# dcjones/polee

Measured on AMD Instinct MI355X. Metric: approx-lik VI iters/sec, higher is better.
Workload: dtype f32

## Files before the change

include/polee_hip_debug.h:

```cpp
#ifndef POLEE_HIP_DEBUG_H
#define POLEE_HIP_DEBUG_H

#include "polee_hip.h"

#ifdef __cplusplus
extern "C" {
#endif

polee_status polee_debug_ptt_plan(const int32_t *node_parent_idxs, const int32_t *node_js, int32_t N,
                                  uint32_t *tour_code, int32_t *tour_tgt, int32_t *leaf_tid,
                                  int32_t *lo, int32_t *mid, int32_t *hi1, int32_t *max_depth);

typedef struct polee_psell_debug polee_psell_debug;
typedef struct {
    int64_t m, n, nnz, num_slices, num_tiles, padded_nnz, num_empty_rows;
    int64_t data_bytes, dict_len;
    int32_t max_row_nnz, max_tile_cols;
    const uint8_t *data;
    const uint32_t *slice_off;
    const uint32_t *tile_slice;
    const uint32_t *tile_dict;
    const uint32_t *dict;
    const uint32_t *row_order;
    const float *slice_ks;
    const uint8_t *slice_flags;
    int64_t num_tiles_a;
    int64_t num_tiles_a1;
    int64_t num_tiles_a1m;
    int64_t num_tiles_a2;
    const uint8_t *slice_w;
    int64_t num_tiles_s;
    int64_t stream_rows[8], stream_nnz[8], stream_bytes[8];
    int64_t csr_num_rows;
    const uint32_t *csr_rowptr;
    const uint32_t *csr_col;
    const float *csr_val;
    const uint32_t *csr_rows;
    int64_t single_num_rows;
    const uint32_t *single_rows;
    const float *single_cnt;
    double single_logsum;
} polee_psell_view;
polee_status polee_debug_psell_build(int64_t m, int64_t n, const void *colptr, int colptr_bytes,
                                     const uint32_t *rowval, const float *nzval,
                                     const int64_t *ks_or_null, polee_psell_debug **out);
polee_status polee_debug_psell_build_device(polee_ctx *ctx, int64_t m, int64_t n, const void *colptr, int colptr_bytes,
                                            const uint32_t *rowval, const float *nzval, const int64_t *ks_or_null,
                                            int device_stages, polee_psell_debug **out);
polee_status polee_debug_psell_view(const polee_psell_debug *p, polee_psell_view *view);
void polee_debug_psell_free(polee_psell_debug *p);

void polee_debug_device_cache_poison(int64_t *checked_blocks, int64_t *bad_blocks, int64_t *bad_words);

polee_status polee_debug_loglik_force_mixed(polee_loglik *ll, int on);

int64_t polee_debug_regression_num_stats(const polee_regression *reg);
polee_status polee_debug_regression_data_pass(polee_regression *reg, const float *noise, float *stats);
polee_status polee_debug_regression_prior_pass(polee_regression *reg, const float *stats, float *loss,
                                               float *grad_or_null);

polee_status polee_debug_comm_allreduce_ms(polee_comm *comm, int64_t count, int32_t reps, double *ms_avg);

polee_status polee_debug_fast_log(polee_ctx *ctx, const double *x, int64_t count, double *out);
polee_status polee_debug_fast_exp(polee_ctx *ctx, const double *x, int64_t count, double *out);

polee_status polee_debug_gibbs_assignments(polee_gibbs *g, int32_t chain, int32_t *z);

polee_status polee_debug_binomial(polee_ctx *ctx, const int64_t *N, const double *p, int64_t count, uint64_t seed, int64_t *out);

polee_status polee_debug_kmer_edges_count(polee_ctx *ctx_or_null, int64_t n, const uint64_t *sketches, int64_t *count);
polee_status polee_debug_kmer_edges_fill(polee_ctx *ctx_or_null, int64_t n, const uint64_t *sketches, int64_t capacity,
                                         uint32_t *u, uint32_t *v, uint32_t *mat, uint32_t *empt);

#ifdef __cplusplus
}
#endif
#endif
```

polee_amd/csrc/vi.hip:

```cpp
#include "loglik_internal.hpp"
#include "ptt_internal.hpp"
#include "vi_fused.hpp"
#include "comm_internal.hpp"
#include "rng.hpp"
#include "sampler_internal.hpp"

#include <cmath>

namespace polee {

struct NoiseSrc {
    const float *z0;
    uint64_t seed;
    int32_t K;
    int64_t nm1;
    __device__ inline float get(int step , int d, int64_t k) const
    {
        if (z0) return z0[((int64_t)(step - 1) * K + d) * nm1 + k];
        return philox_randn(seed, (uint32_t)step, (uint32_t)d, (uint32_t)k);
    }
    template <int KK>
    __device__ inline void get_all(int step, int64_t k, float (&z)[KK]) const
    {
        if (z0) {
#pragma unroll
            for (int d = 0; d < KK; ++d) z[d] = z0[((int64_t)(step - 1) * K + d) * nm1 + k];
            return;
        }
#pragma unroll
        for (int g = 0; g < (KK + 3) / 4; ++g) {
            float q[4];
            philox_randn4(seed, (uint32_t)step, (uint32_t)g, (uint32_t)k, q);
#pragma unroll
            for (int e = 0; e < 4; ++e)
                if (4 * g + e < KK) z[4 * g + e] = q[e];
        }
    }
};

__device__ inline float logistic_f32(float x) { return 1.0f / (1.0f + expf(-x)); }

__global__ void vi_trace_kernel(const double *lp, const double *ladj_el, const double *row_sums, int K, int idx,
                                double *elbo_trace, double *lp_trace)
{
    if (threadIdx.x != 0 || blockIdx.x != 0) return;
    const int d = K - 1;
    elbo_trace[idx] = (lp[d] + ladj_el[d * 2 + 0] + ladj_el[d * 2 + 1] + row_sums[d * 2 + 1]) / K;
    double s = 0.0;
    for (int i = 0; i < K; ++i) s += lp[i];
    lp_trace[idx] = s / K;
}

__global__ void vi_init_mu_kernel(const double *ys, int64_t nm1, float *mu, float *omega, float *alpha)
{
    const int64_t k = (int64_t)blockIdx.x * blockDim.x + threadIdx.x;
    if (k >= nm1) return;
    const double y = ys[k];
    mu[k] = (float)log(y / (1 - y));
    omega[k] = logf(0.1f);
    alpha[k] = 0.0f;
}

__global__ void aos_to_rows_f32_kernel(const float *in, int K, int64_t n, float *out, const uint32_t *index_of)
{
    const int64_t i = (int64_t)blockIdx.x * blockDim.x + threadIdx.x;
    if (i >= n * K) return;
    const int k = (int)(i / n);
    const int64_t j = i - (int64_t)k * n;
    out[i] = in[(index_of ? (int64_t)index_of[j] : j) * K + k];
}

__global__ void remap_u32_kernel(const uint32_t *src, const uint32_t *map, int64_t count, uint32_t *dst)
{
    const int64_t i = (int64_t)blockIdx.x * blockDim.x + threadIdx.x;
    if (i < count) dst[i] = map[src[i]];
}
template <typename T>
__global__ void gather_kernel(const T *src, const int32_t *idx, int64_t count, T *dst)
{
    const int64_t i = (int64_t)blockIdx.x * blockDim.x + threadIdx.x;
    if (i < count) dst[i] = src[idx[i]];
}

__global__ void vi_xgrad_rows_kernel(const float *g, const float *efflens, const double *csum, GenePrior gp, int K,
                                     int64_t n, double *out, const uint32_t *index_of)
{
    const int64_t i = (int64_t)blockIdx.x * blockDim.x + threadIdx.x;
    if (i >= n * K) return;
    const int k = (int)(i / n);
    const int64_t tid = index_of ? (int64_t)index_of[i - (int64_t)k * n] : i - (int64_t)k * n;
    double xg = (double)g[tid * K + k];
    if (efflens) xg -= (double)((float)n * (1.0f / efflens[tid])) / csum[k];
    if (gp.gene_of) {
        const int gene = gp.gene_of[tid];
        const int kg = gene >= 0 ? gp.gene_k[gene] : 0;
        const double c = csum[k], inv_l = (double)(1.0f / efflens[tid]);
        const double xlg = kg > 1 ? -(double)(kg - 1) / gp.gene_c[(size_t)gene * K + k] : 0.0;
        xg += xlg * (inv_l / c) + inv_l * (gp.M / (c * c));
    }
    out[i] = xg;
}

struct UniformLeafLoad {
    double val;
    __device__ dd operator()(int, int64_t) const { return dd_make(val); }
};
__global__ void vi_inverse_nodes_kernel(PttView v, const dd *C, double *ys)
{
    const int k = blockIdx.x * blockDim.x + threadIdx.x;
    if (k >= v.n - 1) return;
    const int lo = v.lo[k], mid = v.mid[k], hi1 = v.hi1[k];
    const double ur = dd_diff(C[mid], C[lo]);
    const double ul = dd_diff(C[hi1], C[mid]);
    ys[k] = ul / (ul + ur);
}

__global__ void sampler_y_kernel(const float *mu, const float *sigma, const float *alpha, NoiseSrc noise, int d_off, double y_eps,
                                 double *ys)
{
    const int64_t k = (int64_t)blockIdx.x * blockDim.x + threadIdx.x;
    const int d = blockIdx.y;
    if (k >= noise.nm1) return;
    const float z0 = noise.get(1, noise.z0 ? d : d + d_off, k);
    const float zs = sinhf(alpha[k] + asinhf(z0));
    double y = (double)logistic_f32(mu[k] + zs * sigma[k]);
    if (y_eps > 0.0) y = y < y_eps ? y_eps : (y > 1 - y_eps ? 1 - y_eps : y);
    ys[(int64_t)d * noise.nm1 + k] = y;
}

__global__ void export_noise_kernel(NoiseSrc noise, int step, float *out)
{
    const int64_t k = (int64_t)blockIdx.x * blockDim.x + threadIdx.x;
    const int d = blockIdx.y;
    if (k < noise.nm1) out[(int64_t)d * noise.nm1 + k] = noise.get(step, d, k);
}

}

using namespace polee;

struct polee_vi {
    polee_ctx *ctx = nullptr;
    polee_loglik *ll = nullptr;
    polee_ptt *t = nullptr;
    polee_vi_opts o;
    int32_t n = 0, K = 0;
    int32_t step = 0;
    int32_t ahead_step = 0;
    int32_t trace_cap = 0;
    polee_comm *comm = nullptr;
    DevBuf<float> d_efflens, d_mu, d_omega, d_alpha, d_mm, d_vm, d_mo, d_vo, d_ma, d_va, d_z0, d_x, d_g;
    DevBuf<float> d_zcur;
    DevBuf<float> d_y32;
    DevBuf<float> d_u32;
    DevBuf<uint32_t> d_open_ptr, d_open_code;
    bool leaf_order = false;
    DevBuf<uint32_t> d_index_of, d_dict_leaf, d_csr_col_leaf;
    DevBuf<float> d_single_leaf;
    LoglikRemap remap{nullptr, nullptr, nullptr, nullptr, false};
    DevBuf<double> d_ys, d_lyy, d_uleaf, d_part_c, d_part_ladj, d_csum, d_lp, d_ladj_el, d_rows, d_elbo, d_lptrace;
    DevBuf<dd> d_C;
    DevBuf<dd> d_chunk_bu;
    DevBuf<int32_t> d_node_start;
    DevBuf<uint32_t> d_need;
    DevBuf<float> d_H;
    int32_t bu_ch = 0;
    DevBuf<int> d_flag;
    DevBuf<int32_t> d_gene_of;
    DevBuf<int> d_gene_k;
    DevBuf<double> d_gene_c;
    int32_t num_genes = 0;
    double gene_M = 0.0;
    DevBuf<double> d_ygrad, d_xgrad_rows;
    DevBuf<float> d_mug, d_omg, d_alg, d_x_rows;

    NoiseSrc noise() const { return NoiseSrc{d_z0.p, o.seed, K, (int64_t)n - 1}; }
    polee_status one_step(bool apply, bool want_values, bool hook_outputs);
};

template <int K>
static polee_status vi_step_k(polee_vi *vi, bool apply, bool want_values, bool hook_outputs)
{
    polee_ctx *ctx = vi->ctx;
    polee_ptt *t = vi->t;
    const polee_vi_opts &o = vi->o;
    const int32_t n = vi->n;
    const int64_t nm1 = n - 1;
    const int step_num = vi->step + 1;
    hipStream_t st = ctx->stream;
    const PttView view = t->view();
    PttView lview = view;
    if (vi->leaf_order) lview.leaf_tid = nullptr;
    const LoglikRemap *remap = vi->leaf_order ? &vi->remap : nullptr;
    const uint32_t *index_of = vi->leaf_order ? vi->d_index_of.p : nullptr;
    const int nch_f = fwd_num_chunks(t->TL);
    const float *eff = o.use_efflen_jacobian ? vi->d_efflens.p : nullptr;
    VK<K> *chunk_f = reinterpret_cast<VK<K> *>(t->d_chunk.p);
    const NoiseSrc noise = vi->noise();

    if (want_values) POLEE_HIP_TRY(ctx, hipMemsetAsync(vi->d_ladj_el.p, 0, sizeof(double) * K * 2, st));
    if (nm1 > 0 && (vi->ahead_step != step_num || want_values)) {
        hipLaunchKernelGGL((vi_sample_k_kernel<K, NoiseSrc>), dim3((unsigned)ceil_div(nm1, 256)), dim3(256), 0, st,
                           vi->d_mu.p, vi->d_omega.p, vi->d_alpha.p, noise, step_num, vi->d_y32.p,
                           vi->d_zcur.p, want_values ? vi->d_ladj_el.p : nullptr);
        POLEE_KERNEL_CHECK(ctx);
    }
    const int own_f = nch_f <= 2048;
    const YRows ysrc{vi->d_y32.p, o.y_eps};
    const bool open_lists = vi->d_open_ptr.p != nullptr;
    static const bool xwin_fold = getenv("POLEE_VI_XWIN_FOLD") != nullptr && getenv("POLEE_NO_RING") == nullptr;
    const bool xwin_here = xwin_fold && !vi->leaf_order && !vi->ll->force_mixed && vi->ll->d_xwin.p && vi->ll->d_tslot_ptr.p && vi->ll->host.num_tiles_s > 0;
    if (open_lists) {
    } else if (nch_f > 1) {
        hipLaunchKernelGGL((vi_fwd_reduce_kernel<K, YRows>), dim3(nch_f), dim3(SCAN_THREADS), 0, st, view, ysrc, chunk_f);
        if (!own_f) hipLaunchKernelGGL((scan_spine_kernel<VK<K>>), dim3(1), dim3(SCAN_THREADS), 0, st, chunk_f, nch_f);
    } else {
        POLEE_HIP_TRY(ctx, hipMemsetAsync(chunk_f, 0, sizeof(VK<K>), st));
    }
    if (want_values) {
        hipLaunchKernelGGL((vi_fwd_apply_kernel<K, YRows, float, true>), dim3(nch_f), dim3(SCAN_THREADS), 0, st, lview, ysrc, chunk_f,
                           vi->d_u32.p, vi->d_x.p, vi->d_g.p, eff, (float)o.y_eps, (float)(1.0 - o.y_eps),
                           eff ? vi->d_part_c.p : nullptr, want_values ? vi->d_part_ladj.p : nullptr, nch_f > 1 ? own_f : 0,
                           (const uint32_t *)vi->d_open_ptr.p, (const uint32_t *)vi->d_open_code.p,
                           xwin_here ? (const uint32_t *)vi->ll->d_tslot_ptr.p : nullptr, xwin_here ? (const uint32_t *)vi->ll->d_tslot.p : nullptr,
                           xwin_here ? vi->ll->d_xwin.p : nullptr,
                           remap && remap->singles_in_g ? (const float *)vi->d_single_leaf.p : nullptr);
    } else {
        hipLaunchKernelGGL((vi_fwd_apply_kernel<K, YRows, float, false>), dim3(nch_f), dim3(SCAN_THREADS), 0, st, lview, ysrc, chunk_f,
                           vi->d_u32.p, vi->d_x.p, vi->d_g.p, eff, (float)o.y_eps, (float)(1.0 - o.y_eps),
                           eff ? vi->d_part_c.p : nullptr, want_values ? vi->d_part_ladj.p : nullptr, nch_f > 1 ? own_f : 0,
                           (const uint32_t *)vi->d_open_ptr.p, (const uint32_t *)vi->d_open_code.p,
                           xwin_here ? (const uint32_t *)vi->ll->d_tslot_ptr.p : nullptr, xwin_here ? (const uint32_t *)vi->ll->d_tslot.p : nullptr,
                           xwin_here ? vi->ll->d_xwin.p : nullptr,
                           remap && remap->singles_in_g ? (const float *)vi->d_single_leaf.p : nullptr);
    }
    POLEE_KERNEL_CHECK(ctx);
    if (want_values) POLEE_HIP_TRY(ctx, hipMemsetAsync(vi->d_lp.p, 0, sizeof(double) * PSELL_MAX_K, st));
    {
        const bool det_saved = vi->ll->deterministic;
        if (o.deterministic > 0 || (o.deterministic == 0 && vi->comm && vi->comm->nranks > 1)) vi->ll->deterministic = true;
        vi->ll->side_part = eff ? vi->d_part_c.p : nullptr;
        vi->ll->side_nparts = nch_f;
        vi->ll->side_out = vi->d_csum.p;
        vi->ll->side_done = false;
        const polee_status ls = loglik_eval_device(vi->ll, vi->d_x.p, K, vi->d_g.p, want_values ? vi->d_lp.p : nullptr, xwin_here, remap);
        vi->ll->deterministic = det_saved;
        const bool side_done = vi->ll->side_done;
        vi->ll->side_part = nullptr;
        POLEE_TRY(ls);
        if (eff && !side_done)
            hipLaunchKernelGGL((vi_csum_finish_kernel<K>), dim3(1), dim3(256), 0, st, (const double *)vi->d_part_c.p, nch_f, vi->d_csum.p);
    }
    if (vi->comm) {
        POLEE_TRY(comm_allreduce_device(vi->comm, vi->d_g.p, (size_t)n * K, false));
        if (want_values) POLEE_TRY(comm_allreduce_device(vi->comm, vi->d_lp.p, (size_t)K, true));
    }
    GenePrior gp{nullptr, nullptr, nullptr, 0.0};
    if (vi->num_genes > 0) {
        gp = GenePrior{vi->d_gene_of.p, vi->d_gene_k.p, vi->d_gene_c.p, vi->gene_M};
        POLEE_HIP_TRY(ctx, hipMemsetAsync(vi->d_gene_c.p, 0, sizeof(double) * (size_t)vi->num_genes * K, st));
        hipLaunchKernelGGL((vi_gene_sums_kernel<K>), dim3((unsigned)ceil_div((int64_t)n, 256)), dim3(256), 0, st, vi->d_x.p,
                           vi->d_efflens.p, vi->d_part_c.p, nch_f, (int64_t)n, gp, vi->d_gene_c.p);
    }
    AdamConsts a;
    a.lr = std::max(o.adam_min_learning_rate,
                    o.adam_initial_learning_rate * std::exp(-o.adam_learning_rate_decay * (double)(step_num - 1)));
    a.rm = o.adam_rm;
    a.rv = o.adam_rv;
    a.eps = o.adam_eps;
    a.m_denom = 1 - std::pow(o.adam_rm, (double)step_num);
    a.v_denom = 1 - std::pow(o.adam_rv, (double)step_num);
    a.inv_m_denom = 1.0 / a.m_denom;
    a.inv_v_denom = 1.0 / a.v_denom;
    a.max_mu = o.max_mu_step;
    a.max_omega = o.max_omega_step;
    a.max_alpha = o.max_alpha_step;
    a.first = step_num == 1;
    const bool sample_next = apply && !(o.z0 && step_num + 1 > o.num_steps);
    const UpdArgs ua{vi->d_y32.p, vi->d_mu.p, vi->d_omega.p, vi->d_alpha.p, vi->d_mm.p, vi->d_vm.p, vi->d_mo.p, vi->d_vo.p,
                     vi->d_ma.p, vi->d_va.p, a, apply ? 1 : 0, vi->d_flag.p, hook_outputs ? vi->d_ygrad.p : nullptr,
                     hook_outputs ? vi->d_mug.p : nullptr, hook_outputs ? vi->d_omg.p : nullptr,
                     hook_outputs ? vi->d_alg.p : nullptr, sample_next ? 1 : 0, o.y_eps, vi->d_zcur.p, step_num};
    {
        const int nch_bu = (int)ceil_div((int64_t)n, bu_ch<K>());
        VD<K> *chunk_bu = reinterpret_cast<VD<K> *>(vi->d_chunk_bu.p);
        const BwdArgs<K> ba{lview, vi->d_u32.p, vi->d_g.p, eff, vi->d_csum.p, gp, chunk_bu, vi->d_C.p, (const uint32_t *)vi->d_need.p,
                            (const int32_t *)vi->d_node_start.p, vi->d_H.p};
        hipLaunchKernelGGL((vi_bwd_local_kernel<K>), dim3(nch_bu), dim3(256), 0, st, ba);
        if (nm1 > 0) {
            hipLaunchKernelGGL((vi_bwd_spine_kernel<K>), dim3(1), dim3(64 * K), 0, st, chunk_bu, nch_bu);
            hipLaunchKernelGGL((vi_update_k_kernel<K, NoiseSrc>), dim3((unsigned)ceil_div(nm1, 256)), dim3(256), 0, st, view,
                               (const float *)vi->d_H.p, (const VD<K> *)chunk_bu, (const dd *)vi->d_C.p, ua, noise);
        }
        if (nm1 > 0) vi->ahead_step = apply ? (sample_next ? step_num + 1 : 0) : step_num;
    }
    POLEE_KERNEL_CHECK(ctx);
    if (want_values) {
        hipLaunchKernelGGL((vi_values_finish_kernel<K>), dim3(1), dim3(256), 0, st, vi->d_part_ladj.p, nch_f,
                           eff ? vi->d_csum.p : nullptr, vi->d_rows.p);
        POLEE_KERNEL_CHECK(ctx);
    }
    if (hook_outputs) {
        hipLaunchKernelGGL(vi_xgrad_rows_kernel, dim3((unsigned)ceil_div((int64_t)n * K, 256)), dim3(256), 0, st,
                           vi->d_g.p, eff, vi->d_csum.p, gp, K, (int64_t)n, vi->d_xgrad_rows.p, index_of);
        POLEE_KERNEL_CHECK(ctx);
    }
    if (want_values && apply && vi->step < vi->trace_cap) {
        hipLaunchKernelGGL(vi_trace_kernel, dim3(1), dim3(64), 0, st, vi->d_lp.p, vi->d_ladj_el.p, vi->d_rows.p, K,
                           vi->step, vi->d_elbo.p, vi->d_lptrace.p);
        POLEE_KERNEL_CHECK(ctx);
    }
    if (apply) ++vi->step;
    return POLEE_OK;
}

polee_status polee_vi::one_step(bool apply, bool want_values, bool hook_outputs)
{
    POLEE_TRY(t->reserve(K));
    if (o.z0 && step + 1 > o.num_steps)
        return fail(ctx, POLEE_ERR_BAD_ARG, "caller-supplied z0 covers only %d steps", o.num_steps);
    switch (K) {
        case 1: return vi_step_k<1>(this, apply, want_values, hook_outputs);
        case 2: return vi_step_k<2>(this, apply, want_values, hook_outputs);
        case 3: return vi_step_k<3>(this, apply, want_values, hook_outputs);
        case 4: return vi_step_k<4>(this, apply, want_values, hook_outputs);
        case 5: return vi_step_k<5>(this, apply, want_values, hook_outputs);
        case 6: return vi_step_k<6>(this, apply, want_values, hook_outputs);
        case 7: return vi_step_k<7>(this, apply, want_values, hook_outputs);
        case 8: return vi_step_k<8>(this, apply, want_values, hook_outputs);
    }
    return fail(ctx, POLEE_ERR_BAD_ARG, "num_mc_samples must be in 1..8");
}

namespace polee {

static polee_status sampler_draw_device(polee_ptt *t, const float *mu, const float *sigma, const float *alpha,
                                        const float *z0, int32_t ndraws, uint64_t seed, DevBuf<float> &d_all,
                                        double y_eps = 0.0)
{
    polee_ctx *ctx = t->ctx;
    if (!mu || !sigma || !alpha || ndraws < 1) return fail(ctx, POLEE_ERR_BAD_ARG, "bad argument");
    if (t->T != 1) return fail(ctx, POLEE_ERR_BAD_ARG, "the sampler needs a single tree");
    const size_t n = t->n, nm1 = n - 1;
    DevBuf<float> d_mu, d_sigma, d_alpha, d_z0;
    POLEE_TRY(d_mu.upload(ctx, mu, nm1));
    POLEE_TRY(d_sigma.upload(ctx, sigma, nm1));
    POLEE_TRY(d_alpha.upload(ctx, alpha, nm1));
    POLEE_TRY(d_all.alloc(ctx, (size_t)ndraws * n));
    for (int32_t b0 = 0; b0 < ndraws; b0 += SAMPLER_BLOCK) {
        const int32_t B = std::min(SAMPLER_BLOCK, ndraws - b0);
        if (z0) POLEE_TRY(d_z0.upload(ctx, z0 + (size_t)b0 * nm1, (size_t)B * nm1));
        POLEE_TRY(sampler_block_device(t, d_mu.p, d_sigma.p, d_alpha.p, z0 ? d_z0.p : nullptr, seed, (uint64_t)b0, 0, B, y_eps,
                                       d_all.p + (size_t)b0 * n, (int64_t)n));
    }
    return POLEE_OK;
}

polee_status sampler_block_device(polee_ptt *t, const float *d_mu, const float *d_sigma, const float *d_alpha, const float *d_z0,
                                  uint64_t seed, uint64_t b0, int32_t r0, int32_t B, double y_eps, float *d_xs, int64_t xs_rs)
{
    polee_ctx *ctx = t->ctx;
    const size_t nm1 = (size_t)t->n - 1;
    POLEE_TRY(t->reserve(B));
    NoiseSrc noise{d_z0, sampler_block_seed(seed, b0), B, (int64_t)nm1};
    if (nm1 > 0) {
        hipLaunchKernelGGL(sampler_y_kernel, dim3((unsigned)ceil_div(nm1, 256), B), dim3(256), 0, ctx->stream, d_mu, d_sigma,
                           d_alpha, noise, (int)r0, y_eps, t->d_ys.p);
        POLEE_KERNEL_CHECK(ctx);
    }
    FwdOut o;
    o.xs = d_xs;
    o.xs_rs = xs_rs;
    return ptt_forward_device(t, t->d_ys.p, B, o);
}

__global__ void sampler_mean_kernel(const float *xs, int ndraws, int64_t n, float *pm)
{
    const int64_t j = (int64_t)blockIdx.x * blockDim.x + threadIdx.x;
    if (j >= n) return;
    float acc = 0.0f;
    for (int k = 0; k < ndraws; ++k) acc += fminf(fmaxf(xs[(int64_t)k * n + j], 1e-15f), 0.9999999f);
    pm[j] = acc / (float)ndraws;
}

__global__ void x0_sums_kernel(const float *xs, const float *efflens, int64_t n, double *sums)
{
    __shared__ double smd[4];
    const int d = blockIdx.y;
    double q = 0.0;
    for (int64_t j = (int64_t)blockIdx.x * blockDim.x + threadIdx.x; j < n; j += (int64_t)gridDim.x * blockDim.x)
        q += (double)(xs[(int64_t)d * n + j] / efflens[j]);
    q = block_sum_f64(q, smd);
    if (threadIdx.x == 0) atomicAdd(&sums[d], q);
}
__global__ void x0_mean_kernel(const float *xs, const float *efflens, const double *sums, int ndraws, int64_t n, float *x0)
{
    const int64_t j = (int64_t)blockIdx.x * blockDim.x + threadIdx.x;
    if (j >= n) return;
    float acc = 0.0f;
    for (int d = 0; d < ndraws; ++d) acc += (xs[(int64_t)d * n + j] / efflens[j]) / (float)sums[d];
    x0[j] = acc / (float)ndraws;
}

constexpr int SAMPLER_MAX_Q = 8;
struct QuantileSpec {
    int nq;
    int j[SAMPLER_MAX_Q];
    double gamma[SAMPLER_MAX_Q];
};
__global__ __launch_bounds__(64) void sampler_quantile_kernel(const float *xs, int ndraws, int64_t n, QuantileSpec spec,
                                                              int in_lds, float *out)
{
    extern __shared__ float col[];
    const int64_t jj = (int64_t)blockIdx.x * 64 + threadIdx.x;
    const int64_t j = jj < n ? jj : n - 1;
    if (in_lds)
        for (int k = 0; k < ndraws; ++k) col[k * 64 + threadIdx.x] = xs[(int64_t)k * n + j];
    auto at = [&](int k) { return in_lds ? col[k * 64 + threadIdx.x] : xs[(int64_t)k * n + j]; };
    float a[SAMPLER_MAX_Q], b[SAMPLER_MAX_Q];
#pragma unroll
    for (int i = 0; i < SAMPLER_MAX_Q; ++i) a[i] = b[i] = 0.0f;
    for (int e = 0; e < ndraws; ++e) {
        const float ve = at(e);
        int rank = 0;
        for (int i = 0; i < ndraws; ++i) {
            const float vi = at(i);
            rank += (vi < ve || (vi == ve && i < e)) ? 1 : 0;
        }
#pragma unroll
        for (int i = 0; i < SAMPLER_MAX_Q; ++i)
            if (i < spec.nq) {
                if (rank == spec.j[i] - 1) a[i] = ve;
                if (rank == spec.j[i] || ndraws == 1) b[i] = ve;
            }
    }
    if (jj < n)
#pragma unroll
        for (int i = 0; i < SAMPLER_MAX_Q; ++i)
            if (i < spec.nq) out[(int64_t)i * n + j] = (float)((double)a[i] + spec.gamma[i] * (double)(b[i] - a[i]));
}

}
using namespace polee;

extern "C" {

void polee_vi_default_opts(polee_vi_opts *o)
{
    if (!o) return;
    memset(o, 0, sizeof(*o));
    o->num_steps = 500;
    o->num_mc_samples = 6;
    o->use_efflen_jacobian = 1;
    o->gradonly = 1;
    o->seed = 123456789ull;
    o->z0 = nullptr;
    o->y_eps = 1e-10;
    o->adam_initial_learning_rate = 1.0;
    o->adam_learning_rate_decay = 2e-2;
    o->adam_min_learning_rate = 1e-3;
    o->adam_eps = 1e-8;
    o->adam_rv = 0.9;
    o->adam_rm = 0.7;
    o->max_mu_step = 2e-1;
    o->max_omega_step = 2e-1;
    o->max_alpha_step = 2e-2;
    o->profile = 0;
    o->deterministic = 0;
    o->gene_of = nullptr;
}

static thread_local bool g_vi_plain_order = false;

polee_status polee_vi_create(polee_loglik *ll, polee_ptt *t, const float *efflens, const polee_vi_opts *opts,
                             polee_vi **out)
{
    if (!ll || !t) return fail(nullptr, POLEE_ERR_BAD_ARG, "null handle");
    polee_ctx *ctx = ll->ctx;
    POLEE_TRY(use_device(ctx));
    if (t->ctx != ctx) return fail(ctx, POLEE_ERR_BAD_ARG, "likelihood and tree belong to different contexts");
    if (!out || !efflens) return fail(ctx, POLEE_ERR_BAD_ARG, "null argument");
    if (t->T != 1) return fail(ctx, POLEE_ERR_BAD_ARG, "the VI loop needs a single tree");
    if ((int64_t)t->n != ll->n)
        return fail(ctx, POLEE_ERR_BAD_ARG, "tree has %d leaves but X has %lld transcripts", t->n, (long long)ll->n);
    polee_vi_opts o;
    if (opts)
        o = *opts;
    else
        polee_vi_default_opts(&o);
    if (o.num_mc_samples < 1 || o.num_mc_samples > PSELL_MAX_K)
        return fail(ctx, POLEE_ERR_BAD_ARG, "num_mc_samples must be in 1..8");
    if (o.num_steps < 0) return fail(ctx, POLEE_ERR_BAD_ARG, "num_steps must be >= 0");
    if (!(o.y_eps > 0.0 && o.y_eps < 0.5)) return fail(ctx, POLEE_ERR_BAD_ARG, "y_eps must lie in (0, 0.5) (LIKAP_Y_EPS = 1e-10)");
    std::vector<int> gene_k;
    double gene_M = 0.0;
    if (o.gene_of) {
        if (!o.use_efflen_jacobian)
            return fail(ctx, POLEE_ERR_BAD_ARG, "gene_of needs use_efflen_jacobian (gene_noninformative_prior! works on the "
                                                "xls of the effective-length adjustment, likelihood.jl:114-159)");
        int32_t ng = 0;
        for (int64_t i = 0; i < ll->n; ++i) {
            if (o.gene_of[i] < -1) return fail(ctx, POLEE_ERR_BAD_ARG, "gene_of[%lld] = %d", (long long)i, o.gene_of[i]);
            ng = std::max(ng, o.gene_of[i] + 1);
        }
        gene_k.assign((size_t)ng, 0);
        for (int64_t i = 0; i < ll->n; ++i)
            if (o.gene_of[i] >= 0) ++gene_k[o.gene_of[i]];
        for (int k : gene_k)
            if (k > 1) gene_M += (double)(k - 1);
    }
    polee_vi *vi = new (std::nothrow) polee_vi();
    if (!vi) return fail(ctx, POLEE_ERR_OOM, "out of host memory");
    vi->ctx = ctx;
    vi->ll = ll;
    vi->t = t;
    ctx_retain(ctx);
    loglik_retain(ll);
    ptt_retain(t);
    vi->o = o;
    vi->n = t->n;
    vi->K = o.num_mc_samples;
    ll->profile = o.profile != 0;
    ll->prof_every = o.profile > 1 ? o.profile : 1;
    const size_t n = vi->n, nm1 = std::max<size_t>(n - 1, 1), K = vi->K;
    polee_status s = POLEE_OK;
    auto A = [&](polee_status r) {
        if (s == POLEE_OK) s = r;
    };
    A(vi->d_efflens.upload(ctx, efflens, n));
    for (DevBuf<float> *b : {&vi->d_mu, &vi->d_omega, &vi->d_alpha, &vi->d_mm, &vi->d_vm, &vi->d_mo, &vi->d_vo,
                             &vi->d_ma, &vi->d_va, &vi->d_mug, &vi->d_omg, &vi->d_alg})
        A(b->alloc(ctx, nm1));
    A(vi->d_x.alloc(ctx, n * K));
    A(vi->d_zcur.alloc(ctx, nm1 * K));
    A(vi->d_y32.alloc(ctx, nm1 * K));
    A(vi->d_g.alloc(ctx, n * K));
    A(vi->d_x_rows.alloc(ctx, n * K));
    A(vi->d_ys.alloc(ctx, nm1));
    if (g_vi_plain_order) A(vi->d_lyy.alloc(ctx, nm1 * 2));
    A(vi->d_u32.alloc(ctx, n * K));
    if (g_vi_plain_order) A(vi->d_uleaf.alloc(ctx, n));
    A(vi->d_C.alloc(ctx, (n + 1) * K));
    {
        const size_t nch = (size_t)std::max(scan_num_chunks(3 * (int64_t)n - 2), 1);
        A(vi->d_part_c.alloc(ctx, nch * K));
        A(vi->d_part_ladj.alloc(ctx, nch * K));
        A(vi->d_csum.alloc(ctx, 2 * PSELL_MAX_K));
    }
    {
        const PttPlan &pl = t->plans[0];
        const int CH = K <= 6 ? bu_ch<6>() : bu_ch<8>();
        vi->bu_ch = CH;
        const int nch_bu = (int)ceil_div((int64_t)n, CH);
        std::vector<int32_t> node_start((size_t)nch_bu + 1, (int32_t)(n - 1));
        std::vector<uint32_t> need((n + 1 + 31) / 32 + 1, 0u);
        bool monotone = true;
        int c = 0;
        for (size_t k = 0; k + 1 < n; ++k) {
            if (k > 0 && pl.lo[k] < pl.lo[k - 1]) monotone = false;
            for (; c <= pl.lo[k] / CH; ++c) node_start[(size_t)c] = (int32_t)k;
            const int64_t end = std::min<int64_t>(((int64_t)pl.lo[k] / CH + 1) * CH, (int64_t)n);
            if (pl.hi1[k] > end)
                for (int32_t b : {pl.lo[k], pl.mid[k], pl.hi1[k]}) need[(size_t)b >> 5] |= 1u << (b & 31);
        }
        if (!monotone) A(fail(ctx, POLEE_ERR_BAD_ARG, "tree plan: internal nodes are not in DFS pre-order"));
        A(vi->d_node_start.upload(ctx, node_start));
        A(vi->d_need.upload(ctx, need));
        A(vi->d_chunk_bu.alloc(ctx, ((size_t)nch_bu + 1) * K));
        A(vi->d_H.alloc(ctx, 2 * K * nm1));
        if (s == POLEE_OK && hipMemsetAsync(vi->d_C.p, 0, sizeof(dd) * (n + 1) * K, ctx->stream) != hipSuccess)
            A(fail(ctx, POLEE_ERR_HIP, "memset failed"));
    }
    {
        static const bool no_open = getenv("POLEE_VI_NO_OPEN_LISTS") != nullptr;
        const std::vector<uint32_t> &code = t->plans[0].tour_code;
        const int64_t TL = t->TL;
        const size_t limit = (size_t)8 << 20;
        std::vector<uint32_t> optr, ocode;
        const bool ok = !no_open && t->T == 1 && (int64_t)code.size() == TL && build_open_lists(code.data(), TL, FWD_CHUNK, limit, optr, ocode);
        if (ok) {
            if (ocode.empty()) ocode.push_back(4u | TOUR_LEAF);
            A(vi->d_open_ptr.upload(ctx, optr));
            A(vi->d_open_code.upload(ctx, ocode));
        }
    }
    A(vi->d_ygrad.alloc(ctx, nm1 * K));
    A(vi->d_xgrad_rows.alloc(ctx, n * K));
    A(vi->d_lp.alloc(ctx, PSELL_MAX_K));
    A(vi->d_ladj_el.alloc(ctx, PSELL_MAX_K * 2));
    A(vi->d_rows.alloc(ctx, PSELL_MAX_K * 2));
    A(vi->d_flag.alloc(ctx, 1));
    if (!gene_k.empty()) {
        vi->num_genes = (int32_t)gene_k.size();
        vi->gene_M = gene_M;
        A(vi->d_gene_of.upload(ctx, o.gene_of, n));
        A(vi->d_gene_k.upload(ctx, gene_k));
        A(vi->d_gene_c.alloc(ctx, gene_k.size() * K));
    }
    static const bool no_leaf_env = getenv("POLEE_VI_NO_LEAF_ORDER") != nullptr;
    if (!no_leaf_env && !g_vi_plain_order && n > 1 && t->plans.size() == 1 && t->plans[0].tid_pos.size() == n) {
        const PttPlan &pl = t->plans[0];
        std::vector<uint32_t> index_of(n);
        std::vector<float> eff_leaf(n);
        for (size_t j = 0; j < n; ++j) index_of[j] = (uint32_t)pl.tid_pos[j];
        for (size_t pos = 0; pos < n; ++pos) eff_leaf[pos] = efflens[pl.leaf_tid[pos]];
        A(vi->d_index_of.upload(ctx, index_of));
        A(vi->d_efflens.upload(ctx, eff_leaf));
        if (!gene_k.empty()) {
            std::vector<int32_t> gene_leaf(n);
            for (size_t pos = 0; pos < n; ++pos) gene_leaf[pos] = o.gene_of[pl.leaf_tid[pos]];
            A(vi->d_gene_of.upload(ctx, gene_leaf));
        }
        A(vi->d_dict_leaf.alloc(ctx, (size_t)std::max<int64_t>(ll->dict_len, 1)));
        if (ll->csr_nnz > 0) A(vi->d_csr_col_leaf.alloc(ctx, (size_t)ll->csr_nnz));
        if (ll->has_singles) A(vi->d_single_leaf.alloc(ctx, n));
        if (s == POLEE_OK) {
            hipStream_t st0 = ctx->stream;
            if (ll->dict_len > 0)
                hipLaunchKernelGGL(remap_u32_kernel, dim3((unsigned)ceil_div(ll->dict_len, 256)), dim3(256), 0, st0,
                                   (const uint32_t *)ll->d_dict.p, (const uint32_t *)vi->d_index_of.p, ll->dict_len, vi->d_dict_leaf.p);
            if (ll->csr_nnz > 0)
                hipLaunchKernelGGL(remap_u32_kernel, dim3((unsigned)ceil_div(ll->csr_nnz, 256)), dim3(256), 0, st0,
                                   (const uint32_t *)ll->d_csr_col.p, (const uint32_t *)vi->d_index_of.p, ll->csr_nnz, vi->d_csr_col_leaf.p);
            if (ll->has_singles)
                hipLaunchKernelGGL(gather_kernel<float>, dim3((unsigned)ceil_div((int64_t)n, 256)), dim3(256), 0, st0,
                                   (const float *)ll->d_single_cnt.p, (const int32_t *)t->d_leaf_tid.p, (int64_t)n, vi->d_single_leaf.p);
            if (hipGetLastError() != hipSuccess) A(fail(ctx, POLEE_ERR_HIP, "leaf-order tables: kernel launch failed"));
            vi->leaf_order = true;
            vi->remap = LoglikRemap{vi->d_dict_leaf.p, ll->has_singles ? vi->d_single_leaf.p : nullptr,
                                    ll->csr_nnz > 0 ? vi->d_csr_col_leaf.p : nullptr, vi->d_index_of.p, ll->has_singles};
        }
    }
    vi->o.gene_of = nullptr;
    vi->trace_cap = o.gradonly ? 0 : std::max(o.num_steps, 1);
    if (!o.gradonly) {
        A(vi->d_elbo.alloc(ctx, vi->trace_cap));
        A(vi->d_lptrace.alloc(ctx, vi->trace_cap));
    }
    if (o.z0 && o.num_steps > 0) A(vi->d_z0.upload(ctx, o.z0, (size_t)o.num_steps * K * (n - 1)));
    vi->o.z0 = o.z0;
    A(t->reserve((int32_t)K));
    if (s != POLEE_OK) {
        polee_vi_destroy(vi);
        return s;
    }
    hipStream_t st = ctx->stream;
    hipError_t e = hipMemsetAsync(vi->d_flag.p, 0, sizeof(int), st);
    if (e == hipSuccess) e = hipMemsetAsync(vi->d_rows.p, 0, sizeof(double) * PSELL_MAX_K * 2, st);
    for (DevBuf<float> *b : {&vi->d_mm, &vi->d_vm, &vi->d_mo, &vi->d_vo, &vi->d_ma, &vi->d_va})
        if (e == hipSuccess) e = hipMemsetAsync(b->p, 0, sizeof(float) * nm1, st);
    if (e != hipSuccess) {
        polee_vi_destroy(vi);
        return fail(ctx, POLEE_ERR_HIP, "memset failed: %s", hipGetErrorString(e));
    }
    if (n > 1) {
        UniformLeafLoad load{(double)(1.0f / (float)n)};
        LeafPrefixEmit emit{(int32_t)n, t->d_C.p};
        e = run_scan_partial<dd>(st, 1, n, t->d_chunk.p, nullptr, load, emit);
        if (e == hipSuccess) {
            hipLaunchKernelGGL(vi_inverse_nodes_kernel, dim3((unsigned)ceil_div(n - 1, 256)), dim3(256), 0, st,
                               t->view(), t->d_C.p, vi->d_ys.p);
            hipLaunchKernelGGL(vi_init_mu_kernel, dim3((unsigned)ceil_div(n - 1, 256)), dim3(256), 0, st, vi->d_ys.p,
                               (int64_t)n - 1, vi->d_mu.p, vi->d_omega.p, vi->d_alpha.p);
            e = hipGetLastError();
        }
        if (e == hipSuccess) e = hipStreamSynchronize(st);
        if (e != hipSuccess) {
            polee_vi_destroy(vi);
            return fail(ctx, POLEE_ERR_HIP, "initialisation failed: %s", hipGetErrorString(e));
        }
    }
    *out = vi;
    return POLEE_OK;
}

void polee_vi_destroy(polee_vi *vi)
{
    if (!vi) return;
    polee_ctx *ctx = vi->ctx;
    polee_loglik *ll = vi->ll;
    polee_ptt *t = vi->t;
    polee_comm *comm = vi->comm;
    if (ctx) {
        (void)hipSetDevice(ctx->device);
        (void)hipStreamSynchronize(ctx->stream);
    }
    delete vi;
    polee_comm_destroy(comm);
    loglik_release(ll);
    ptt_release(t);
    ctx_release(ctx);
}

polee_status polee_vi_set_comm(polee_vi *vi, polee_comm *comm)
{
    if (!vi) return fail(nullptr, POLEE_ERR_BAD_ARG, "null handle");
    if (comm && comm->ctx != vi->ctx)
        return fail(vi->ctx, POLEE_ERR_BAD_ARG, "communicator and fit belong to different contexts");
    if (comm) ++comm->refs;
    polee_comm_destroy(vi->comm);
    vi->comm = comm;
    return POLEE_OK;
}

polee_status polee_vi_run(polee_vi *vi, int32_t nsteps)
{
    if (!vi) return fail(nullptr, POLEE_ERR_BAD_ARG, "null handle");
    POLEE_TRY(use_device(vi->ctx));
    vi->ll->profile = vi->o.profile != 0;
    vi->ll->prof_every = vi->o.profile > 1 ? vi->o.profile : 1;
    for (int32_t i = 0; i < nsteps; ++i) POLEE_TRY(vi->one_step(true, !vi->o.gradonly, false));
    return POLEE_OK;
}

polee_status polee_vi_sync(polee_vi *vi)
{
    if (!vi) return fail(nullptr, POLEE_ERR_BAD_ARG, "null handle");
    polee_ctx *ctx = vi->ctx;
    POLEE_TRY(use_device(ctx));
    int flag = 0;
    POLEE_TRY(vi->d_flag.download(ctx, &flag, 1));
    if (vi->ll->profile) POLEE_TRY(vi->ll->profile_collect());
    if (flag != 0)
        return fail(ctx, POLEE_ERR_NONFINITE, "non-finite gradient at VI step %d (likelihood-approximation.jl:559)",
                    flag);
    return POLEE_OK;
}

polee_status polee_vi_get_params(polee_vi *vi, float *mu, float *omega, float *alpha)
{
    if (!vi) return fail(nullptr, POLEE_ERR_BAD_ARG, "null handle");
    polee_ctx *ctx = vi->ctx;
    POLEE_TRY(use_device(ctx));
    const size_t nm1 = vi->n - 1;
    if (mu) POLEE_TRY(vi->d_mu.download(ctx, mu, nm1));
    if (omega) POLEE_TRY(vi->d_omega.download(ctx, omega, nm1));
    if (alpha) POLEE_TRY(vi->d_alpha.download(ctx, alpha, nm1));
    return POLEE_OK;
}

polee_status polee_vi_set_params(polee_vi *vi, const float *mu, const float *omega, const float *alpha)
{
    if (!vi) return fail(nullptr, POLEE_ERR_BAD_ARG, "null handle");
    polee_ctx *ctx = vi->ctx;
    POLEE_TRY(use_device(ctx));
    const size_t nm1 = vi->n - 1;
    if (mu) POLEE_TRY(vi->d_mu.upload(ctx, mu, nm1));
    if (omega) POLEE_TRY(vi->d_omega.upload(ctx, omega, nm1));
    if (alpha) POLEE_TRY(vi->d_alpha.upload(ctx, alpha, nm1));
    vi->ahead_step = 0;
    return POLEE_OK;
}

polee_status polee_vi_get_stats(polee_vi *vi, polee_vi_stats *stats)
{
    if (!vi || !stats) return fail(nullptr, POLEE_ERR_BAD_ARG, "null argument");
    polee_ctx *ctx = vi->ctx;
    POLEE_TRY(use_device(ctx));
    memset(stats, 0, sizeof(*stats));
    stats->steps_done = vi->step;
    int flag = 0;
    POLEE_TRY(vi->d_flag.download(ctx, &flag, 1));
    stats->nonfinite_step = flag;
    if (vi->ll->profile) POLEE_TRY(vi->ll->profile_collect());
    stats->loglik_kernel_launches = vi->ll->prof_launches;
    stats->loglik_kernel_ms_avg = vi->ll->prof_launches ? vi->ll->prof_ms_total / vi->ll->prof_launches : 0.0;
    stats->loglik_pass_ms_avg = vi->ll->prof_launches ? vi->ll->prof_pass_ms_total / vi->ll->prof_launches : 0.0;
    if (!vi->o.gradonly && vi->step > 0 && vi->step <= vi->trace_cap) {
        POLEE_HIP_TRY(ctx, hipMemcpyAsync(&stats->last_elbo, vi->d_elbo.p + (vi->step - 1), sizeof(double),
                                          hipMemcpyDeviceToHost, ctx->stream));
        POLEE_HIP_TRY(ctx, hipMemcpyAsync(&stats->last_lp_mean, vi->d_lptrace.p + (vi->step - 1), sizeof(double),
                                          hipMemcpyDeviceToHost, ctx->stream));
        POLEE_HIP_TRY(ctx, hipStreamSynchronize(ctx->stream));
    }
    return POLEE_OK;
}

polee_status polee_vi_get_trace(polee_vi *vi, double *elbo, double *lp_mean)
{
    if (!vi) return fail(nullptr, POLEE_ERR_BAD_ARG, "null handle");
    polee_ctx *ctx = vi->ctx;
    POLEE_TRY(use_device(ctx));
    if (vi->o.gradonly) return fail(ctx, POLEE_ERR_BAD_ARG, "no trace is recorded in gradonly mode");
    const size_t cnt = std::min(vi->step, vi->trace_cap);
    if (elbo) POLEE_TRY(vi->d_elbo.download(ctx, elbo, cnt));
    if (lp_mean) POLEE_TRY(vi->d_lptrace.download(ctx, lp_mean, cnt));
    return POLEE_OK;
}

#ifdef POLEE_VI_STAMPS
polee_status polee_debug_vi_stamps(unsigned long long *out)
{
    return hipMemcpyFromSymbol(out, HIP_SYMBOL(polee::g_vi_stamps), sizeof(unsigned long long) * 4 * 2048 * 8) == hipSuccess ? POLEE_OK : POLEE_ERR_HIP;
}
#endif

polee_status polee_vi_export_noise(polee_vi *vi, int32_t step, float *z0)
{
    if (!vi || !z0 || step < 1) return fail(nullptr, POLEE_ERR_BAD_ARG, "bad argument");
    polee_ctx *ctx = vi->ctx;
    POLEE_TRY(use_device(ctx));
    const int64_t nm1 = vi->n - 1;
    if (nm1 < 1) return POLEE_OK;
    if (vi->o.z0 && step > vi->o.num_steps) return fail(ctx, POLEE_ERR_BAD_ARG, "step beyond the supplied noise");
    DevBuf<float> tmp;
    POLEE_TRY(tmp.alloc(ctx, (size_t)vi->K * nm1));
    hipLaunchKernelGGL(export_noise_kernel, dim3((unsigned)ceil_div(nm1, 256), vi->K), dim3(256), 0, ctx->stream,
                       vi->noise(), step, tmp.p);
    POLEE_KERNEL_CHECK(ctx);
    return tmp.download(ctx, z0, (size_t)vi->K * nm1);
}

polee_status polee_vi_eval_gradients(polee_vi *vi, float *xs, double *x_grad, double *y_grad, float *mu_grad,
                                     float *omega_grad, float *alpha_grad, double *lp, double *ladj)
{
    if (!vi) return fail(nullptr, POLEE_ERR_BAD_ARG, "null handle");
    polee_ctx *ctx = vi->ctx;
    POLEE_TRY(use_device(ctx));
    const size_t n = vi->n, nm1 = n - 1, K = vi->K;
    POLEE_TRY(vi->one_step(false, true, true));
    if (xs) {
        hipLaunchKernelGGL(aos_to_rows_f32_kernel, dim3((unsigned)ceil_div(n * K, 256)), dim3(256), 0, ctx->stream,
                           vi->d_x.p, (int)K, (int64_t)n, vi->d_x_rows.p, vi->leaf_order ? (const uint32_t *)vi->d_index_of.p : nullptr);
        POLEE_KERNEL_CHECK(ctx);
        POLEE_TRY(vi->d_x_rows.download(ctx, xs, n * K));
    }
    if (x_grad) POLEE_TRY(vi->d_xgrad_rows.download(ctx, x_grad, n * K));
    if (y_grad) POLEE_TRY(vi->d_ygrad.download(ctx, y_grad, nm1 * K));
    if (mu_grad) POLEE_TRY(vi->d_mug.download(ctx, mu_grad, nm1));
    if (omega_grad) POLEE_TRY(vi->d_omg.download(ctx, omega_grad, nm1));
    if (alpha_grad) POLEE_TRY(vi->d_alg.download(ctx, alpha_grad, nm1));
    if (lp) POLEE_TRY(vi->d_lp.download(ctx, lp, K));
    if (ladj) {
        std::vector<double> el(K * 2), rs(K * 2);
        POLEE_TRY(vi->d_ladj_el.download(ctx, el.data(), K * 2));
        POLEE_TRY(vi->d_rows.download(ctx, rs.data(), K * 2));
        for (size_t d = 0; d < K; ++d) ladj[d] = el[d * 2] + el[d * 2 + 1] + rs[d * 2 + 1];
    }
    return POLEE_OK;
}

polee_status polee_vi_fit(polee_loglik *ll, polee_ptt *t, const float *efflens, const polee_vi_opts *opts, float *mu,
                          float *omega, float *alpha, polee_vi_stats *stats)
{
    polee_vi *vi = nullptr;
    POLEE_TRY(polee_vi_create(ll, t, efflens, opts, &vi));
    polee_status s = polee_vi_run(vi, vi->o.num_steps);
    if (s == POLEE_OK) s = polee_vi_sync(vi);
    if (s == POLEE_OK) s = polee_vi_get_params(vi, mu, omega, alpha);
    if (s == POLEE_OK && stats) s = polee_vi_get_stats(vi, stats);
    polee_vi_destroy(vi);
    return s;
}

polee_status polee_optimize_ptt(polee_loglik *ll, polee_ptt *t, const float *efflens, int32_t num_steps, float *xs,
                                float *zs_out)
{
    if (!ll || !t || !efflens || !xs || num_steps < 0) return fail(nullptr, POLEE_ERR_BAD_ARG, "bad argument");
    polee_vi_opts o;
    polee_vi_default_opts(&o);
    o.num_steps = num_steps;
    o.num_mc_samples = 1;
    polee_vi *vi = nullptr;
    g_vi_plain_order = true;
    const polee_status cs = polee_vi_create(ll, t, efflens, &o, &vi);
    g_vi_plain_order = false;
    POLEE_TRY(cs);
    polee_ctx *ctx = vi->ctx;
    hipStream_t st = ctx->stream;
    const int32_t n = vi->n;
    const int64_t nm1 = n - 1;
    const PttView view = t->view();
    const int nch_f = fwd_num_chunks(t->TL), nch_b = scan_num_chunks(n);
    VK<1> *chunk_f = reinterpret_cast<VK<1> *>(t->d_chunk.p);
    VD<1> *chunk_b = reinterpret_cast<VD<1> *>(t->d_chunk.p);
    polee_status rc = POLEE_OK;
    auto forward = [&]() -> polee_status {
        hipLaunchKernelGGL(point_sample_kernel, dim3((unsigned)ceil_div(nm1, 256)), dim3(256), 0, st, vi->d_mu.p, nm1,
                           vi->d_ys.p, vi->d_lyy.p);
        if (nch_f > 1) {
            hipLaunchKernelGGL((vi_fwd_reduce_kernel<1, LogRows>), dim3(nch_f), dim3(SCAN_THREADS), 0, st, view, LogRows{vi->d_lyy.p}, chunk_f);
            hipLaunchKernelGGL((scan_spine_kernel<VK<1>>), dim3(1), dim3(SCAN_THREADS), 0, st, chunk_f, nch_f);
        } else {
            POLEE_HIP_TRY(ctx, hipMemsetAsync(chunk_f, 0, sizeof(VK<1>), st));
        }
        hipLaunchKernelGGL((vi_fwd_apply_kernel<1, LogRows, double, false>), dim3(nch_f), dim3(SCAN_THREADS), 0, st, view, LogRows{vi->d_lyy.p}, chunk_f,
                           vi->d_uleaf.p, vi->d_x.p, vi->d_g.p, vi->d_efflens.p, (float)o.y_eps, (float)(1.0 - o.y_eps),
                           vi->d_part_c.p, (double *)nullptr, 0, (const uint32_t *)nullptr, (const uint32_t *)nullptr,
                           (const uint32_t *)nullptr, (const uint32_t *)nullptr, (float *)nullptr, (const float *)nullptr);
        POLEE_KERNEL_CHECK(ctx);
        return POLEE_OK;
    };
    for (int step_num = 1; step_num <= num_steps && rc == POLEE_OK && nm1 > 0; ++step_num) {
        rc = forward();
        if (rc != POLEE_OK) break;
        rc = loglik_eval_device(ll, vi->d_x.p, 1, vi->d_g.p, nullptr);
        if (rc != POLEE_OK) break;
        const GenePrior no_gp{nullptr, nullptr, nullptr, 0.0};
        hipLaunchKernelGGL((vi_bwd_reduce_kernel<1>), dim3(nch_b), dim3(SCAN_THREADS), 0, st, view, vi->d_uleaf.p,
                           vi->d_g.p, vi->d_efflens.p, vi->d_part_c.p, nch_f, vi->d_csum.p, no_gp, chunk_b);
        hipLaunchKernelGGL((scan_spine_kernel<VD<1>>), dim3(1), dim3(SCAN_THREADS), 0, st, chunk_b, nch_b);
        hipLaunchKernelGGL((vi_bwd_apply_kernel<1>), dim3(nch_b), dim3(SCAN_THREADS), 0, st, view, vi->d_uleaf.p,
                           vi->d_g.p, vi->d_efflens.p, vi->d_csum.p, no_gp, chunk_b, vi->d_C.p, 0);
        AdamConsts a;
        a.lr = std::max(o.adam_min_learning_rate,
                        o.adam_initial_learning_rate * std::exp(-o.adam_learning_rate_decay * (double)(step_num - 1)));
        a.rm = o.adam_rm;
        a.rv = o.adam_rv;
        a.eps = o.adam_eps;
        a.m_denom = 1 - std::pow(o.adam_rm, (double)step_num);
        a.v_denom = 1 - std::pow(o.adam_rv, (double)step_num);
        a.inv_m_denom = 1.0 / a.m_denom;
        a.inv_v_denom = 1.0 / a.v_denom;
        a.max_mu = 1e-1;
        a.max_omega = a.max_alpha = 0.0;
        a.first = step_num == 1;
        hipLaunchKernelGGL(point_update_kernel, dim3((unsigned)ceil_div(nm1, 256)), dim3(256), 0, st, view, vi->d_ys.p,
                           vi->d_C.p, vi->d_mu.p, vi->d_mm.p, vi->d_vm.p, a, vi->d_flag.p, step_num);
        hipError_t e = hipGetLastError();
        if (e != hipSuccess) rc = fail(ctx, POLEE_ERR_HIP, "kernel launch failed: %s", hipGetErrorString(e));
    }
    if (rc == POLEE_OK) rc = forward();
    if (rc == POLEE_OK) rc = polee_vi_sync(vi);
    if (rc == POLEE_OK) rc = vi->d_x.download(ctx, xs, n);
    if (rc == POLEE_OK && zs_out) rc = vi->d_mu.download(ctx, zs_out, nm1);
    polee_vi_destroy(vi);
    return rc;
}

polee_status polee_sampler_draw(polee_ptt *t, const float *mu, const float *sigma, const float *alpha,
                                const float *z0, int32_t ndraws, uint64_t seed, float *xs)
{
    if (!t) return fail(nullptr, POLEE_ERR_BAD_ARG, "null tree");
    polee_ctx *ctx = t->ctx;
    POLEE_TRY(use_device(ctx));
    if (!xs) return fail(ctx, POLEE_ERR_BAD_ARG, "bad argument");
    DevBuf<float> d_all;
    POLEE_TRY(sampler_draw_device(t, mu, sigma, alpha, z0, ndraws, seed, d_all));
    return d_all.download(ctx, xs, (size_t)ndraws * t->n);
}

polee_status polee_sampler_initial_values(polee_ptt *t, const float *mu, const float *sigma, const float *alpha,
                                          const float *efflens, const float *z0, int32_t ndraws, uint64_t seed, float *x0)
{
    if (!t) return fail(nullptr, POLEE_ERR_BAD_ARG, "null tree");
    polee_ctx *ctx = t->ctx;
    POLEE_TRY(use_device(ctx));
    if (!x0 || !efflens) return fail(ctx, POLEE_ERR_BAD_ARG, "bad argument");
    DevBuf<float> d_all, d_l, d_x0;
    DevBuf<double> d_sums;
    POLEE_TRY(sampler_draw_device(t, mu, sigma, alpha, z0, ndraws, seed, d_all, 1e-10 ));
    const int64_t n = t->n;
    POLEE_TRY(d_l.upload(ctx, efflens, (size_t)n));
    POLEE_TRY(d_x0.alloc(ctx, (size_t)n));
    POLEE_TRY(d_sums.alloc(ctx, (size_t)ndraws));
    POLEE_HIP_TRY(ctx, hipMemsetAsync(d_sums.p, 0, sizeof(double) * ndraws, ctx->stream));
    hipLaunchKernelGGL(x0_sums_kernel, dim3((unsigned)std::min<int64_t>(ceil_div(n, 256), 256), (unsigned)ndraws), dim3(256), 0,
                       ctx->stream, d_all.p, d_l.p, n, d_sums.p);
    hipLaunchKernelGGL(x0_mean_kernel, dim3((unsigned)ceil_div(n, 256)), dim3(256), 0, ctx->stream, d_all.p, d_l.p, d_sums.p,
                       ndraws, n, d_x0.p);
    POLEE_KERNEL_CHECK(ctx);
    return d_x0.download(ctx, x0, (size_t)n);
}

polee_status polee_sampler_posterior_mean(polee_ptt *t, const float *mu, const float *sigma, const float *alpha,
                                          const float *z0, int32_t ndraws, uint64_t seed, float *pm)
{
    if (!t) return fail(nullptr, POLEE_ERR_BAD_ARG, "null tree");
    polee_ctx *ctx = t->ctx;
    POLEE_TRY(use_device(ctx));
    if (!pm) return fail(ctx, POLEE_ERR_BAD_ARG, "bad argument");
    DevBuf<float> d_all, d_pm;
    POLEE_TRY(sampler_draw_device(t, mu, sigma, alpha, z0, ndraws, seed, d_all));
    POLEE_TRY(d_pm.alloc(ctx, (size_t)t->n));
    hipLaunchKernelGGL(sampler_mean_kernel, dim3((unsigned)ceil_div(t->n, 256)), dim3(256), 0, ctx->stream, d_all.p,
                       ndraws, (int64_t)t->n, d_pm.p);
    POLEE_KERNEL_CHECK(ctx);
    return d_pm.download(ctx, pm, (size_t)t->n);
}

polee_status polee_sampler_quantiles(polee_ptt *t, const float *mu, const float *sigma, const float *alpha,
                                     const float *z0, int32_t ndraws, uint64_t seed, const double *qs, int32_t nq,
                                     float *quantiles)
{
    if (!t) return fail(nullptr, POLEE_ERR_BAD_ARG, "null tree");
    polee_ctx *ctx = t->ctx;
    POLEE_TRY(use_device(ctx));
    if (!qs || !quantiles || nq < 1 || nq > SAMPLER_MAX_Q) return fail(ctx, POLEE_ERR_BAD_ARG, "1..%d quantiles", SAMPLER_MAX_Q);
    QuantileSpec spec{};
    spec.nq = nq;
    for (int i = 0; i < nq; ++i) {
        if (!(qs[i] >= 0.0 && qs[i] <= 1.0)) return fail(ctx, POLEE_ERR_BAD_ARG, "quantile %g outside [0, 1]", qs[i]);
        const double aleph = (double)(ndraws - 1) * qs[i] + 1.0;
        const int j = ndraws == 1 ? 1 : std::min(std::max((int)aleph, 1), ndraws - 1);
        spec.j[i] = j;
        spec.gamma[i] = std::min(std::max(aleph - j, 0.0), 1.0);
    }
    DevBuf<float> d_all, d_q;
    POLEE_TRY(sampler_draw_device(t, mu, sigma, alpha, z0, ndraws, seed, d_all));
    const int64_t n = t->n;
    POLEE_TRY(d_q.alloc(ctx, (size_t)nq * n));
    const bool in_lds = (size_t)ndraws * 64 * sizeof(float) <= 48 * 1024;
    hipLaunchKernelGGL(sampler_quantile_kernel, dim3((unsigned)ceil_div(n, 64)), dim3(64),
                       in_lds ? (size_t)ndraws * 64 * sizeof(float) : 0, ctx->stream, d_all.p, ndraws, n, spec,
                       in_lds ? 1 : 0, d_q.p);
    POLEE_KERNEL_CHECK(ctx);
    return d_q.download(ctx, quantiles, (size_t)nq * n);
}

}
```

polee_amd/csrc/vi_fused.hpp:

```cpp
#pragma once
#include "ptt_internal.hpp"

namespace polee {

#ifdef POLEE_VI_STAMPS
__device__ unsigned long long g_vi_stamps[4][2048][8];
#define VI_STAMP(kern, slot)                                                                                        \
    do {                                                                                                            \
        asm volatile("s_waitcnt vmcnt(0) lgkmcnt(0)" ::: "memory");                                                 \
        if (threadIdx.x == 0 && blockIdx.x < 2048) g_vi_stamps[kern][blockIdx.x][slot] = __builtin_amdgcn_s_memrealtime(); \
    } while (0)
#else
#define VI_STAMP(kern, slot) do {} while (0)
#endif

template <int K>
struct VK {
    double v[K];
};
template <int K>
struct VD {
    dd v[K];
};
template <int K>
struct ScanOps<VK<K>> {
    __device__ static VK<K> zero()
    {
        VK<K> r;
#pragma unroll
        for (int d = 0; d < K; ++d) r.v[d] = 0.0;
        return r;
    }
    __device__ static VK<K> add(const VK<K> &a, const VK<K> &b)
    {
        VK<K> r;
#pragma unroll
        for (int d = 0; d < K; ++d) r.v[d] = a.v[d] + b.v[d];
        return r;
    }
    __device__ static VK<K> shfl_up(const VK<K> &a, int dist)
    {
        VK<K> r;
#pragma unroll
        for (int d = 0; d < K; ++d) r.v[d] = __shfl_up(a.v[d], dist, 64);
        return r;
    }
    template <int CTRL, int ROW_MASK>
    __device__ static VK<K> dpp(const VK<K> &a)
    {
        VK<K> r;
#pragma unroll
        for (int d = 0; d < K; ++d) r.v[d] = dpp_f64<CTRL, ROW_MASK>(a.v[d]);
        return r;
    }
};
template <int K>
struct ScanOps<VD<K>> {
    __device__ static VD<K> zero()
    {
        VD<K> r;
#pragma unroll
        for (int d = 0; d < K; ++d) r.v[d] = dd{0.0, 0.0};
        return r;
    }
    __device__ static VD<K> add(const VD<K> &a, const VD<K> &b)
    {
        VD<K> r;
#pragma unroll
        for (int d = 0; d < K; ++d) r.v[d] = dd_add(a.v[d], b.v[d]);
        return r;
    }
    __device__ static VD<K> shfl_up(const VD<K> &a, int dist)
    {
        VD<K> r;
#pragma unroll
        for (int d = 0; d < K; ++d) r.v[d] = dd{__shfl_up(a.v[d].hi, dist, 64), __shfl_up(a.v[d].lo, dist, 64)};
        return r;
    }
    template <int CTRL, int ROW_MASK>
    __device__ static VD<K> dpp(const VD<K> &a)
    {
        VD<K> r;
#pragma unroll
        for (int d = 0; d < K; ++d) r.v[d] = dd{dpp_f64<CTRL, ROW_MASK>(a.v[d].hi), dpp_f64<CTRL, ROW_MASK>(a.v[d].lo)};
        return r;
    }
};

template <int K>
__device__ inline void block_sum_vec(double (&v)[K], double *smem)
{
    const int lane = threadIdx.x & 63, wave = threadIdx.x >> 6;
#pragma unroll
    for (int d = 0; d < K; ++d) {
        const double s = wave_inclusive_scan<double>(v[d]);
        if (lane == 63) smem[wave * K + d] = s;
    }
    __syncthreads();
    if (threadIdx.x < K) {
        const double s = smem[threadIdx.x] + smem[K + threadIdx.x] + smem[2 * K + threadIdx.x] + smem[3 * K + threadIdx.x];
        smem[threadIdx.x] = s;
    }
    __syncthreads();
#pragma unroll
    for (int d = 0; d < K; ++d) v[d] = smem[d];
    __syncthreads();
}

template <int K>
__device__ inline void store_vec_by_thread(const double (&v)[K], double *out)
{
#pragma unroll
    for (int d = 0; d < K; ++d)
        if (threadIdx.x == d) out[d] = v[d];
}

__device__ inline float sinh_asinh(float sa, float ca, float z0) { return fmaf(sa, sqrtf(fmaf(z0, z0, 1.0f)), ca * z0); }

__device__ inline double clamped_y(float y32, double y_eps)
{
    const double y = (double)y32;
    return y < y_eps ? y_eps : (y > 1 - y_eps ? 1 - y_eps : y);
}
__device__ inline double clamped_y_pos(float y32, double y_eps, double one_m_eps)
{
    const double y = (double)y32;
    return fmin(fmax(y, y_eps), one_m_eps);
}
template <int K, typename Noise>
__device__ inline void sample_node(float m, float om, float al, const Noise &noise, int step, int64_t k,
                                   float *__restrict__ y32, float *__restrict__ zcur, double *lsum)
{
    const float sigma = expf(om);
    const float sa = sinhf(al), ca = coshf(al);
    float zall[K];
    noise.template get_all<K>(step, k, zall);
#pragma unroll
    for (int d = 0; d < K; ++d) {
        const float z0 = zall[d];
        zcur[k * K + d] = z0;
        const float zs = sinh_asinh(sa, ca, z0);
        const float yf = 1.0f / (1.0f + expf(-(m + zs * sigma)));
        if (lsum) {
            const double y = (double)yf;
            lsum[d] = 0.5 * (double)log1pf(zs * zs) - 0.5 * (double)log1pf(z0 * z0);
            lsum[K + d] = log((double)sigma * y * (1 - y));
        }
        y32[k * K + d] = yf;
    }
}

template <int K, typename Noise>
__global__ __launch_bounds__(256) void vi_sample_k_kernel(const float *__restrict__ mu, const float *__restrict__ omega,
                                                         const float *__restrict__ alpha, Noise noise, int step,
                                                         float *__restrict__ y32, float *__restrict__ zcur,
                                                         double *__restrict__ ladj_out)
{
    __shared__ double smem[4 * 2 * K];
    const int64_t k = (int64_t)blockIdx.x * blockDim.x + threadIdx.x;
    double lsum[2 * K];
#pragma unroll
    for (int d = 0; d < 2 * K; ++d) lsum[d] = 0.0;
    if (k < noise.nm1)
        sample_node<K, Noise>(mu[k], omega[k], alpha[k], noise, step, k, y32, zcur, ladj_out ? lsum : nullptr);
    if (ladj_out) {
        block_sum_vec<2 * K>(lsum, smem);
#pragma unroll
        for (int i = 0; i < 2 * K; ++i)
            if (threadIdx.x == i) atomicAdd(&ladj_out[(i % K) * 2 + i / K], lsum[i]);
    }
}

struct LogRows {
    const double *lyy;
    template <int K>
    __device__ inline double edge_one(uint32_t k, uint32_t left, int d) const { return lyy[((size_t)k * 2 + left) * K + d]; }
    template <int K>
    __device__ inline void edge(uint32_t k, uint32_t left, double (&e)[K]) const
    {
        const double *p = lyy + ((size_t)k * 2 + left) * K;
#pragma unroll
        for (int d = 0; d < K; ++d) e[d] = p[d];
    }
};
struct YRows {
    const float *y32;
    double y_eps;
    template <int K>
    __device__ inline double edge_one(uint32_t k, uint32_t left, int d) const
    {
        const double y = clamped_y_pos(y32[(size_t)k * K + d], y_eps, 1.0 - y_eps);
        return fast_log_pos(left ? y : 1.0 - y);
    }
    template <int K>
    __device__ inline void edge(uint32_t k, uint32_t left, double (&e)[K]) const
    {
        const float *p = y32 + (size_t)k * K;
        const double hi = 1.0 - y_eps;
#pragma unroll
        for (int d = 0; d < K; ++d) {
            const double y = clamped_y_pos(p[d], y_eps, hi);
            e[d] = fast_log_pos(left ? y : 1.0 - y);
        }
    }
};

constexpr int FWD_ITEMS = 2;
constexpr int FWD_CHUNK = SCAN_THREADS * FWD_ITEMS;
inline int fwd_num_chunks(int64_t len) { return (int)((len + FWD_CHUNK - 1) / FWD_CHUNK); }

template <int K, typename Src>
__device__ inline VK<K> tour_value(uint32_t code, const Src &src, VK<K> &edge)
{
    VK<K> val;
    const uint32_t type = code & 3u;
    if (code & 4u) {
#pragma unroll
        for (int d = 0; d < K; ++d) edge.v[d] = 0.0;
    } else {
        src.template edge<K>(code >> 4, (code >> 3) & 1u, edge.v);
    }
#pragma unroll
    for (int d = 0; d < K; ++d) val.v[d] = type == TOUR_ENTER ? edge.v[d] : (type == TOUR_EXIT ? -edge.v[d] : 0.0);
    return val;
}

template <typename T>
__device__ inline T chunk_prefix(const T *__restrict__ chunk_sums, int chunk, T *smem)
{
    T acc = ScanOps<T>::zero();
    for (int i = threadIdx.x; i < chunk; i += SCAN_THREADS) acc = ScanOps<T>::add(acc, chunk_sums[i]);
    T tot;
    (void)block_exclusive_scan<T>(acc, smem, &tot);
    return tot;
}

template <int K, typename Src>
__global__ __launch_bounds__(SCAN_THREADS) void vi_fwd_reduce_kernel(PttView v, Src lyy,
                                                                    VK<K> *__restrict__ chunk_sums)
{
    __shared__ VK<K> smem[SCAN_THREADS / 64];
    const int64_t base = (int64_t)blockIdx.x * FWD_CHUNK + (int64_t)threadIdx.x * FWD_ITEMS;
    VK<K> acc = ScanOps<VK<K>>::zero(), edge;
#pragma unroll
    for (int j = 0; j < FWD_ITEMS; ++j)
        if (base + j < v.TL) acc = ScanOps<VK<K>>::add(acc, tour_value<K, Src>(v.tour_code[base + j], lyy, edge));
    VK<K> tot;
    (void)block_exclusive_scan<VK<K>>(acc, smem, &tot);
    if (threadIdx.x == 0) chunk_sums[blockIdx.x] = tot;
}

template <int K, typename Src, typename UT, bool LADJ>
__global__ __launch_bounds__(SCAN_THREADS) void vi_fwd_apply_kernel(PttView v, Src lyy,
                                                                   const VK<K> *__restrict__ chunk_offsets,
                                                                   UT *__restrict__ uleaf, float *__restrict__ xs,
                                                                   float *__restrict__ g,
                                                                   const float *__restrict__ efflens, float clamp_lo,
                                                                   float clamp_hi, double *__restrict__ part_c,
                                                                   double *__restrict__ part_ladj, int own_prefix,
                                                                   const uint32_t *__restrict__ open_ptr,
                                                                   const uint32_t *__restrict__ open_code,
                                                                   const uint32_t *__restrict__ tslot_ptr,
                                                                   const uint32_t *__restrict__ tslot,
                                                                   float *__restrict__ xwin,
                                                                   const float *__restrict__ single_cnt)
{
    __shared__ VK<K> smem[SCAN_THREADS / 64];
    __shared__ double smd[4 * K];
    __shared__ double spre[K];
    __shared__ double smd2[LADJ ? 4 * K : 1];
    constexpr int XW_INLINE = 12, XW_DEFER = 48;
    __shared__ uint32_t xw_tid[XW_DEFER];
    __shared__ float xw_val[XW_DEFER][K];
    __shared__ int xw_count;
    if (xwin && threadIdx.x == 0) xw_count = 0;
    if (xwin) __syncthreads();
    const int64_t base = (int64_t)blockIdx.x * FWD_CHUNK + (int64_t)threadIdx.x * FWD_ITEMS;
    VK<K> w[FWD_ITEMS];
    uint32_t code[FWD_ITEMS];
    int tgt[FWD_ITEMS];
#pragma unroll
    for (int j = 0; j < FWD_ITEMS; ++j) {
        code[j] = base + j < v.TL ? v.tour_code[base + j] : (4u | TOUR_LEAF);
        tgt[j] = base + j < v.TL ? v.tour_tgt[base + j] : 0;
    }
    VI_STAMP(0, 0);
    const int lane = threadIdx.x & 63;
    uint32_t ob = 0, oe = 0;
    if (open_ptr) {
        ob = open_ptr[blockIdx.x];
        oe = open_ptr[blockIdx.x + 1];
    }
    const int wave = threadIdx.x >> 6;
    const uint32_t ocode0 = ob + lane < oe ? open_code[ob + lane] : (4u | TOUR_LEAF);
    VK<K> acc = ScanOps<VK<K>>::zero();
    float inv_l_[FWD_ITEMS], sc_[FWD_ITEMS];
    int ltid[FWD_ITEMS];
#pragma unroll
    for (int j = 0; j < FWD_ITEMS; ++j) {
        acc = ScanOps<VK<K>>::add(acc, tour_value<K, Src>(code[j], lyy, w[j]));
        const bool leaf = (code[j] & 3u) == TOUR_LEAF && base + j < v.TL;
        ltid[j] = leaf ? (v.leaf_tid ? v.leaf_tid[tgt[j]] : tgt[j]) : 0;
        inv_l_[j] = leaf && efflens ? 1.0f / efflens[ltid[j]] : 0.0f;
        sc_[j] = leaf && single_cnt ? single_cnt[ltid[j]] : 0.0f;
    }
    VI_STAMP(0, 1);
    if (open_ptr) {
#pragma unroll
        for (int dd_ = 0; dd_ < (K + 3) / 4; ++dd_) {
            const int d = wave + 4 * dd_;
            if (d < K) {
                double pre = (ocode0 & 4u) ? 0.0 : lyy.template edge_one<K>(ocode0 >> 4, (ocode0 >> 3) & 1u, d);
                for (uint32_t e = ob + 64 + lane; e < oe; e += 64) {
                    const uint32_t oc = open_code[e];
                    pre += lyy.template edge_one<K>(oc >> 4, (oc >> 3) & 1u, d);
                }
                pre = wave_inclusive_scan<double>(pre);
                if (lane == 63) spre[d] = pre;
            }
        }
    }
    VI_STAMP(0, 2);
    VK<K> tot;
    VK<K> off = block_exclusive_scan<VK<K>>(acc, smem, &tot);
    VI_STAMP(0, 3);
    if (open_ptr) {
#pragma unroll
        for (int d = 0; d < K; ++d) off.v[d] += spre[d];
    } else {
        off = ScanOps<VK<K>>::add(own_prefix ? chunk_prefix<VK<K>>(chunk_offsets, blockIdx.x, smem) : chunk_offsets[blockIdx.x], off);
    }
    double pc[K], pl[K];
#pragma unroll
    for (int d = 0; d < K; ++d) pc[d] = pl[d] = 0.0;
#pragma unroll
    for (int j = 0; j < FWD_ITEMS; ++j) {
        const uint32_t tj = code[j] & 3u;
#pragma unroll
        for (int d = 0; d < K; ++d) off.v[d] = tj == TOUR_ENTER ? off.v[d] + w[j].v[d] : (tj == TOUR_EXIT ? off.v[d] - w[j].v[d] : off.v[d]);
        const VK<K> &inc = off;
        if (base + j < v.TL) {
            const uint32_t type = code[j] & 3u;
            if (type == TOUR_LEAF) {
                const int pos = tgt[j];
                const int tid = ltid[j];
                const float inv_l = inv_l_[j];
                const float sc = sc_[j];
#pragma unroll
                for (int d = 0; d < K; ++d) {
                    const double u = fast_exp(inc.v[d] + w[j].v[d]);
                    uleaf[(size_t)pos * K + d] = (UT)u;
                    float x = (float)u;
                    x = (float)fmax((double)x, 1e-16);
                    x = fminf(fmaxf(x, clamp_lo), clamp_hi);
                    xs[(size_t)tid * K + d] = x;
                    g[(size_t)tid * K + d] = sc != 0.0f ? sc / x : 0.0f;
                    pc[d] += (double)(x * inv_l);
                }
                if (xwin) {
                    const uint32_t sb = tslot_ptr[tid], se = tslot_ptr[tid + 1];
                    int q = -1;
                    if (se - sb > (uint32_t)XW_INLINE) q = atomicAdd(&xw_count, 1);
                    if (q >= 0 && q < XW_DEFER) {
                        xw_tid[q] = (uint32_t)tid;
#pragma unroll
                        for (int d = 0; d < K; ++d) xw_val[q][d] = xs[(size_t)tid * K + d];
                    } else {
                        for (uint32_t e = sb; e < se; ++e) {
                            float *w = xwin + (size_t)tslot[e] * K;
#pragma unroll
                            for (int d = 0; d < K; ++d) w[d] = xs[(size_t)tid * K + d];
                        }
                    }
                }
            } else if (LADJ && type == TOUR_ENTER) {
#pragma unroll
                for (int d = 0; d < K; ++d) pl[d] += inc.v[d];
            }
        }
    }
    if (xwin) {
        __syncthreads();
        const int cnt = min(xw_count, XW_DEFER);
        for (int q = 0; q < cnt; ++q) {
            const uint32_t tid = xw_tid[q], sb = tslot_ptr[tid], se = tslot_ptr[tid + 1];
            for (uint32_t e = sb * K + threadIdx.x; e < se * K; e += SCAN_THREADS) {
                const uint32_t slot = e / K, d = e - slot * K;
                xwin[(size_t)tslot[slot] * K + d] = xw_val[q][d];
            }
        }
    }
    VI_STAMP(0, 4);
    if (part_c || LADJ) {
#pragma unroll
        for (int d = 0; d < K; ++d) {
            const double a = wave_inclusive_scan<double>(pc[d]);
            const double b = LADJ ? wave_inclusive_scan<double>(pl[d]) : 0.0;
            if (lane == 63) {
                smd[wave * K + d] = a;
                if (LADJ) smd2[wave * K + d] = b;
            }
        }
        __syncthreads();
        if ((int)threadIdx.x < K) {
            const int d = threadIdx.x;
            if (part_c) part_c[(size_t)blockIdx.x * K + d] = ((smd[d] + smd[K + d]) + smd[2 * K + d]) + smd[3 * K + d];
            if (LADJ) part_ladj[(size_t)blockIdx.x * K + d] = ((smd2[d] + smd2[K + d]) + smd2[2 * K + d]) + smd2[3 * K + d];
        }
    }
    VI_STAMP(0, 5);
}

struct GenePrior {
    const int32_t *gene_of;
    const int *gene_k;
    const double *gene_c;
    double M;
};

template <int K>
__device__ inline void bwd_values(const PttView &v, int64_t pos, const double *__restrict__ uleaf,
                                  const float *__restrict__ g, const float *__restrict__ efflens,
                                  const double *csum, const GenePrior &gp, VD<K> &a)
{
    const int tid = v.leaf_tid ? v.leaf_tid[pos] : (int)pos;
    const float inv_lf = efflens ? 1.0f / efflens[tid] : 0.0f;
    const float nl = (float)v.n * inv_lf;
    int gene = -1, kg = 0;
    if (gp.gene_of) {
        gene = gp.gene_of[tid];
        kg = gene >= 0 ? gp.gene_k[gene] : 0;
    }
#pragma unroll
    for (int d = 0; d < K; ++d) {
        double xg = (double)g[(size_t)tid * K + d];
        if (efflens) xg -= (double)nl / csum[d];
        if (gp.gene_of) {
            const double c = csum[d], inv_l = (double)inv_lf;
            const double xlg = kg > 1 ? -(double)(kg - 1) / gp.gene_c[(size_t)gene * K + d] : 0.0;
            xg += xlg * (inv_l / c) + inv_l * (gp.M / (c * c));
        }
        a.v[d] = dd_make(uleaf[(size_t)pos * K + d] * xg);
    }
}

template <int K>
__global__ __launch_bounds__(256) void vi_gene_sums_kernel(const float *__restrict__ xs, const float *__restrict__ efflens,
                                                          const double *__restrict__ part_c, int nchunks_fwd, int64_t n,
                                                          GenePrior gp, double *__restrict__ gene_c)
{
    __shared__ double smd[4 * K];
    double c[K];
#pragma unroll
    for (int d = 0; d < K; ++d) c[d] = 0.0;
    for (int ch = threadIdx.x; ch < nchunks_fwd; ch += 256)
#pragma unroll
        for (int d = 0; d < K; ++d) c[d] += part_c[(size_t)ch * K + d];
    block_sum_vec<K>(c, smd);
    const int64_t tid = (int64_t)blockIdx.x * 256 + threadIdx.x;
    if (tid >= n) return;
    const int gene = gp.gene_of[tid];
    if (gene < 0 || gp.gene_k[gene] <= 1) return;
    const float inv_l = 1.0f / efflens[tid];
#pragma unroll
    for (int d = 0; d < K; ++d) {
        const float xl = xs[(size_t)tid * K + d] * inv_l;
        atomicAdd(&gene_c[(size_t)gene * K + d], (double)(float)((double)xl / c[d]));
    }
}

template <int K>
__global__ __launch_bounds__(SCAN_THREADS) void vi_bwd_reduce_kernel(PttView v, const double *__restrict__ uleaf,
                                                                    const float *__restrict__ g,
                                                                    const float *__restrict__ efflens,
                                                                    const double *__restrict__ part_c, int nchunks_fwd,
                                                                    double *__restrict__ csum_out, GenePrior gp,
                                                                    VD<K> *__restrict__ chunk_sums)
{
    __shared__ VD<K> smem[SCAN_THREADS / 64];
    __shared__ double smd[4 * K];
    double c[K];
#pragma unroll
    for (int d = 0; d < K; ++d) c[d] = 0.0;
    if (efflens) {
        for (int ch = threadIdx.x; ch < nchunks_fwd; ch += SCAN_THREADS)
#pragma unroll
            for (int d = 0; d < K; ++d) c[d] += part_c[(size_t)ch * K + d];
        block_sum_vec<K>(c, smd);
        if (blockIdx.x == 0) store_vec_by_thread<K>(c, csum_out);
    }
    const int64_t base = (int64_t)blockIdx.x * SCAN_CHUNK + (int64_t)threadIdx.x * SCAN_ITEMS;
    VD<K> acc = ScanOps<VD<K>>::zero(), a;
#pragma unroll
    for (int j = 0; j < SCAN_ITEMS; ++j)
        if (base + j < v.n) {
            bwd_values<K>(v, base + j, uleaf, g, efflens, c, gp, a);
            acc = ScanOps<VD<K>>::add(acc, a);
        }
    VD<K> tot;
    (void)block_exclusive_scan<VD<K>>(acc, smem, &tot);
    if (threadIdx.x == 0) chunk_sums[blockIdx.x] = tot;
}

template <int K>
__global__ __launch_bounds__(SCAN_THREADS) void vi_bwd_apply_kernel(PttView v, const double *__restrict__ uleaf,
                                                                   const float *__restrict__ g,
                                                                   const float *__restrict__ efflens,
                                                                   const double *__restrict__ csum, GenePrior gp,
                                                                   const VD<K> *__restrict__ chunk_offsets,
                                                                   dd *__restrict__ C, int own_prefix)
{
    __shared__ VD<K> smem[SCAN_THREADS / 64];
    double c[K];
#pragma unroll
    for (int d = 0; d < K; ++d) c[d] = efflens ? csum[d] : 1.0;
    const int64_t base = (int64_t)blockIdx.x * SCAN_CHUNK + (int64_t)threadIdx.x * SCAN_ITEMS;
    VD<K> val[SCAN_ITEMS];
    VD<K> acc = ScanOps<VD<K>>::zero();
#pragma unroll
    for (int j = 0; j < SCAN_ITEMS; ++j) {
        if (base + j < v.n)
            bwd_values<K>(v, base + j, uleaf, g, efflens, c, gp, val[j]);
        else
            val[j] = ScanOps<VD<K>>::zero();
        acc = ScanOps<VD<K>>::add(acc, val[j]);
    }
    VD<K> tot;
    VD<K> off = block_exclusive_scan<VD<K>>(acc, smem, &tot);
    off = ScanOps<VD<K>>::add(own_prefix ? chunk_prefix<VD<K>>(chunk_offsets, blockIdx.x, smem) : chunk_offsets[blockIdx.x], off);
#pragma unroll
    for (int j = 0; j < SCAN_ITEMS; ++j) {
        if (base + j < v.n) {
#pragma unroll
            for (int d = 0; d < K; ++d) C[(size_t)(base + j) * K + d] = off.v[d];
        }
        off = ScanOps<VD<K>>::add(off, val[j]);
        if (base + j == v.n - 1) {
#pragma unroll
            for (int d = 0; d < K; ++d) C[(size_t)v.n * K + d] = off.v[d];
        }
    }
}

__device__ inline double fast_rcp(double x)
{
    double r = __builtin_amdgcn_rcp(x);
    r = fma(fma(-x, r, 1.0), r, r);
    r = fma(fma(-x, r, 1.0), r, r);
    return r;
}

struct AdamConsts {
    double lr, rm, rv, eps, m_denom, v_denom;
    double inv_m_denom, inv_v_denom;
    double max_mu, max_omega, max_alpha;
    int first;
};

__device__ inline void adam_one(float &p, float &m, float &v, float grad, const AdamConsts &a, double max_step)
{
    if (a.first) {
        m = grad;
        v = grad * grad;
    } else {
        m = (float)(a.rm * (double)m + (1 - a.rm) * (double)grad);
        v = (float)(a.rv * (double)v + (1 - a.rv) * (double)(grad * grad));
    }
    const double pm = (double)m * a.inv_m_denom, pv = (double)v * a.inv_v_denom;
    double delta = a.lr * pm * fast_rcp(sqrt(pv) + a.eps);
    delta = delta < -max_step ? -max_step : (delta > max_step ? max_step : delta);
    p = (float)((double)p + delta);
}

struct UpdArgs {
    float *y32;
    float *mu, *omega, *alpha, *m_mu, *v_mu, *m_omega, *v_omega, *m_alpha, *v_alpha;
    AdamConsts adam;
    int apply;
    int *nonfinite_step;
    double *y_grad_out;
    float *mu_grad_out, *omega_grad_out, *alpha_grad_out;
    int sample_next;
    double y_eps;
    float *zcur;
    int step;
};

template <int K, typename Noise>
__device__ inline void update_node(const UpdArgs &A, const Noise &noise, int64_t k, int lo, int mid, int hi1, const double (&hr)[K],
                                   const double (&hl)[K])
{
    const int64_t nm1 = noise.nm1;
    const double cnt_r = (double)(mid - lo - 1), cnt_l = (double)(hi1 - mid - 1);
    const float muk = A.mu[k], omk = A.omega[k], alk = A.alpha[k];
    const float sigma = expf(omk), sa = sinhf(alk), ca = coshf(alk);
    float mu_g = 0.f, om_g = 0.f, al_g = 0.f;
    float p_mu = muk, p_om = omk, p_al = alk;
#pragma unroll
    for (int d = 0; d < K; ++d) {
        const double Hr = cnt_r + hr[d];
        const double Hl = cnt_l + hl[d];
        const double y = clamped_y(A.y32[k * K + d], A.y_eps);
        const double dyy = y * (1 - y);
        const double ygd = (Hl * (1 - y) - Hr * y) * fast_rcp(dyy);
        if (A.y_grad_out) A.y_grad_out[(int64_t)d * nm1 + k] = ygd;
        const float yg = (float)ygd;
        const float z0 = A.zcur[k * K + d];
        const float zs = sinh_asinh(sa, ca, z0);
        const float cc = sqrtf(fmaf(zs, zs, 1.0f));
        mu_g = (float)((double)mu_g + dyy * (double)yg);
        mu_g = (float)((double)mu_g + (1 - 2 * y));
        float sg = (float)(dyy * (double)zs * (double)yg);
        sg = (float)((double)sg + ((double)(1.0f / sigma) + (double)zs * (1 - 2 * y)));
        float zg = (float)(dyy * (double)sigma * (double)yg);
        zg = (float)((double)zg + (double)sigma * (1 - 2 * y));
        al_g += cc * zg;
        al_g += zs / cc;
        om_g += sigma * sg;
    }
    VI_STAMP(2, 2);
    mu_g /= (float)K;
    om_g /= (float)K;
    al_g /= (float)K;
    if (A.mu_grad_out) A.mu_grad_out[k] = mu_g;
    if (A.omega_grad_out) A.omega_grad_out[k] = om_g;
    if (A.alpha_grad_out) A.alpha_grad_out[k] = al_g;
    if (A.apply && !(isfinite(mu_g) && isfinite(om_g) && isfinite(al_g))) atomicCAS(A.nonfinite_step, 0, A.step);
    if (A.apply) {
        float p = muk, mm = A.m_mu[k], vv = A.v_mu[k];
        adam_one(p, mm, vv, mu_g, A.adam, A.adam.max_mu);
        A.mu[k] = p; A.m_mu[k] = mm; A.v_mu[k] = vv;
        p_mu = p;
        p = omk; mm = A.m_omega[k]; vv = A.v_omega[k];
        adam_one(p, mm, vv, om_g, A.adam, A.adam.max_omega);
        A.omega[k] = p; A.m_omega[k] = mm; A.v_omega[k] = vv;
        p_om = p;
        p = alk; mm = A.m_alpha[k]; vv = A.v_alpha[k];
        adam_one(p, mm, vv, al_g, A.adam, A.adam.max_alpha);
        A.alpha[k] = p; A.m_alpha[k] = mm; A.v_alpha[k] = vv;
        p_al = p;
    }
    VI_STAMP(2, 3);
    if (A.sample_next) sample_node<K, Noise>(p_mu, p_om, p_al, noise, A.step + 1, k, A.y32, A.zcur, nullptr);
}

template <int K>
__host__ __device__ constexpr int bu_ch() { return K <= 6 ? 512 : 256; }

template <int K>
struct BwdArgs {
    PttView v;
    const float *uleaf;
    const float *g, *efflens;
    const double *csum;
    GenePrior gp;
    VD<K> *chunk_tot;
    dd *C;
    const uint32_t *need;
    const int32_t *node_start;
    float *H;
};

template <int K>
__device__ inline void csum_finish_block(const double *__restrict__ part_c, int nparts, double *__restrict__ out, double *smem )
{
    double c[K];
#pragma unroll
    for (int d = 0; d < K; ++d) c[d] = 0.0;
    for (int ch = threadIdx.x; ch < nparts; ch += 256)
#pragma unroll
        for (int d = 0; d < K; ++d) c[d] += part_c[(size_t)ch * K + d];
    block_sum_vec<K>(c, smem);
#pragma unroll
    for (int d = 0; d < K; ++d)
        if (threadIdx.x == d) {
            out[d] = c[d];
            out[K + d] = 1.0 / c[d];
        }
}
template <int K>
__global__ __launch_bounds__(256) void vi_csum_finish_kernel(const double *__restrict__ part_c, int nparts, double *__restrict__ out)
{
    __shared__ double smd[4 * K];
    csum_finish_block<K>(part_c, nparts, out, smd);
}

template <int K>
__device__ inline void bwd_leaf(const PttView &v, int64_t pos, const float *__restrict__ uleaf, const float *__restrict__ g,
                                const float *__restrict__ efflens, const double *c, const double *inv_c, const GenePrior &gp,
                                double (&a)[K])
{
    const int tid = v.leaf_tid ? v.leaf_tid[pos] : (int)pos;
    const float inv_lf = efflens ? 1.0f / efflens[tid] : 0.0f;
    const float nl = (float)v.n * inv_lf;
    int gene = -1, kg = 0;
    if (gp.gene_of) {
        gene = gp.gene_of[tid];
        kg = gene >= 0 ? gp.gene_k[gene] : 0;
    }
#pragma unroll
    for (int d = 0; d < K; ++d) {
        double xg = (double)g[(size_t)tid * K + d];
        if (efflens) xg -= (double)nl * inv_c[d];
        if (gp.gene_of) {
            const double cc = c[d], inv_l = (double)inv_lf;
            const double xlg = kg > 1 ? -(double)(kg - 1) / gp.gene_c[(size_t)gene * K + d] : 0.0;
            xg += xlg * (inv_l / cc) + inv_l * (gp.M / (cc * cc));
        }
        a[d] = (double)uleaf[(size_t)pos * K + d] * xg;
    }
}

__device__ inline dd two_sum(double a, double b)
{
    const double s = a + b, bb = s - a;
    return dd{s, (a - (s - bb)) + (b - bb)};
}

template <int K>
__global__ __launch_bounds__(256) void vi_bwd_local_kernel(BwdArgs<K> B)
{
    constexpr int CH = bu_ch<K>(), LPT = CH / 256;
    __shared__ dd P[(CH + 1) * K];
    __shared__ VD<K> wtot[4];
    const PttView &v = B.v;
    const int lane = threadIdx.x & 63, wave = threadIdx.x >> 6;
    double c[K], inv_c[K];
#pragma unroll
    for (int d = 0; d < K; ++d) {
        c[d] = B.efflens ? B.csum[d] : 1.0;
        inv_c[d] = B.efflens ? B.csum[K + d] : 1.0;
    }
    VI_STAMP(1, 0);
    const int64_t base = (int64_t)blockIdx.x * CH, p0 = base + (int64_t)threadIdx.x * LPT;
    const int64_t end = min(base + CH, (int64_t)v.n), nm1 = (int64_t)v.n - 1;
    const bool exp0 = p0 <= v.n && ((B.need[p0 >> 5] >> (p0 & 31)) & 1u);
    const bool exp1 = LPT == 2 && p0 + 1 <= v.n && ((B.need[(p0 + 1) >> 5] >> ((p0 + 1) & 31)) & 1u);
    double a[LPT][K];
#pragma unroll
    for (int j = 0; j < LPT; ++j) {
        if (p0 + j < v.n)
            bwd_leaf<K>(v, p0 + j, B.uleaf, B.g, B.efflens, c, inv_c, B.gp, a[j]);
        else
#pragma unroll
            for (int d = 0; d < K; ++d) a[j][d] = 0.0;
    }
    constexpr int PRE = LPT;
    const uint32_t vz = threadIdx.x >> 12;
    const int32_t k0 = B.node_start[blockIdx.x + vz] + (int32_t)threadIdx.x, k1 = B.node_start[blockIdx.x + 1 + vz];
    int32_t kp[PRE];
    int plo[PRE], pmid[PRE], phi[PRE];
#pragma unroll
    for (int i = 0; i < PRE; ++i) {
        kp[i] = k0 + i * 256;
        const bool in = kp[i] < k1;
        plo[i] = in ? v.lo[kp[i]] : 0;
        pmid[i] = in ? v.mid[kp[i]] : 0;
        phi[i] = in ? v.hi1[kp[i]] : 0;
    }
    VD<K> s;
#pragma unroll
    for (int d = 0; d < K; ++d) {
        s.v[d] = dd_make(a[0][d]);
        if constexpr (LPT == 2) s.v[d] = two_sum(a[0][d], a[1][d]);
    }
    VI_STAMP(1, 1);
    const VD<K> inc = wave_inclusive_scan<VD<K>>(s);
    VI_STAMP(1, 2);
    if (lane == 63) wtot[wave] = inc;
    __syncthreads();
    VD<K> off = wave_shift_up_one<VD<K>>(inc);
    for (int w = 0; w < wave; ++w) off = ScanOps<VD<K>>::add(wtot[w], off);
#pragma unroll
    for (int d = 0; d < K; ++d) P[(size_t)(threadIdx.x * LPT) * K + d] = off.v[d];
    if (exp0)
#pragma unroll
        for (int d = 0; d < K; ++d) B.C[(size_t)p0 * K + d] = off.v[d];
    if constexpr (LPT == 2) {
        const int64_t p1 = p0 + 1;
#pragma unroll
        for (int d = 0; d < K; ++d) {
            const dd o1 = dd_add(off.v[d], dd_make(a[0][d]));
            P[(size_t)(threadIdx.x * LPT + 1) * K + d] = o1;
            if (exp1) B.C[(size_t)p1 * K + d] = o1;
        }
    }
    if (threadIdx.x == 255) {
        VD<K> tot;
#pragma unroll
        for (int d = 0; d < K; ++d) {
            tot.v[d] = dd_add(off.v[d], s.v[d]);
            P[(size_t)CH * K + d] = tot.v[d];
        }
        B.chunk_tot[blockIdx.x] = tot;
    }
    VI_STAMP(1, 3);
    __syncthreads();
    VI_STAMP(1, 4);
    auto node = [&](int32_t k, int lo, int mid, int hi1) {
        if (hi1 > end) return;
        const dd *Plo = P + (size_t)(lo - base) * K, *Pmid = P + (size_t)(mid - base) * K, *Phi = P + (size_t)(hi1 - base) * K;
#pragma unroll
        for (int d = 0; d < K; ++d) {
            const dd pm = Pmid[d];
            B.H[(size_t)d * nm1 + k] = (float)dd_diff(pm, Plo[d]);
            B.H[(size_t)(K + d) * nm1 + k] = (float)dd_diff(Phi[d], pm);
        }
    };
#pragma unroll
    for (int i = 0; i < PRE; ++i)
        if (kp[i] < k1) node(kp[i], plo[i], pmid[i], phi[i]);
    for (int32_t k = k0 + PRE * 256; k < k1; k += 256) node(k, v.lo[k], v.mid[k], v.hi1[k]);
    VI_STAMP(1, 5);
}

template <int K>
__global__ __launch_bounds__(64 * K) void vi_bwd_spine_kernel(VD<K> *chunk_tot, int nch)
{
    const int d = threadIdx.x >> 6, lane = threadIdx.x & 63;
    const int per = (nch + 63) / 64;
    const int b = min(lane * per, nch), e = min(b + per, nch);
    constexpr int FAST = 8;
    dd t[FAST];
    dd acc{0.0, 0.0};
    if (per <= FAST) {
#pragma unroll
        for (int i = 0; i < FAST; ++i) t[i] = b + i < e ? chunk_tot[b + i].v[d] : dd{0.0, 0.0};
#pragma unroll
        for (int i = 0; i < FAST; ++i) acc = dd_add(acc, t[i]);
    } else {
        for (int i = b; i < e; ++i) acc = dd_add(acc, chunk_tot[i].v[d]);
    }
    const dd inc = wave_inclusive_scan<dd>(acc);
    dd off = ScanOps<dd>::shfl_up(inc, 1);
    if (lane == 0) off = dd{0.0, 0.0};
    if (per <= FAST) {
#pragma unroll
        for (int i = 0; i < FAST; ++i) {
            if (b + i < e) chunk_tot[b + i].v[d] = off;
            off = dd_add(off, t[i]);
        }
    } else {
        for (int i = b; i < e; ++i) {
            const dd ti = chunk_tot[i].v[d];
            chunk_tot[i].v[d] = off;
            off = dd_add(off, ti);
        }
    }
    if (lane == 63) chunk_tot[nch].v[d] = inc;
}

template <int K, typename Noise>
__global__ __launch_bounds__(256) void vi_update_k_kernel(PttView v, const float *__restrict__ H, const VD<K> *__restrict__ chunk_off,
                                                         const dd *__restrict__ C, UpdArgs A, Noise noise)
{
    constexpr int CH = bu_ch<K>();
    VI_STAMP(2, 0);
    const int64_t k = (int64_t)blockIdx.x * blockDim.x + threadIdx.x, nm1 = (int64_t)v.n - 1;
    if (k >= nm1) return;
    const int lo = v.lo[k], mid = v.mid[k], hi1 = v.hi1[k];
    double hr[K], hl[K];
    if ((int64_t)hi1 <= min(((int64_t)lo / CH + 1) * CH, (int64_t)v.n)) {
#pragma unroll
        for (int d = 0; d < K; ++d) {
            hr[d] = (double)H[(size_t)d * nm1 + k];
            hl[d] = (double)H[(size_t)(K + d) * nm1 + k];
        }
    } else {
        const dd *Plo = C + (size_t)lo * K, *Pmid = C + (size_t)mid * K, *Phi = C + (size_t)hi1 * K;
        const dd *Olo = chunk_off[lo / CH].v, *Omid = chunk_off[mid / CH].v, *Ohi = chunk_off[hi1 / CH].v;
#pragma unroll
        for (int d = 0; d < K; ++d) {
            const dd gm = dd_add(Omid[d], Pmid[d]);
            hr[d] = dd_diff(gm, dd_add(Olo[d], Plo[d]));
            hl[d] = dd_diff(dd_add(Ohi[d], Phi[d]), gm);
        }
    }
    VI_STAMP(2, 1);
    update_node<K, Noise>(A, noise, k, lo, mid, hi1, hr, hl);
    VI_STAMP(2, 6);
}

__global__ void point_sample_kernel(const float *__restrict__ zs, int64_t nm1, double *__restrict__ ys,
                                    double *__restrict__ lyy)
{
    const int64_t k = (int64_t)blockIdx.x * blockDim.x + threadIdx.x;
    if (k >= nm1) return;
    double y = (double)(1.0f / (1.0f + expf(-zs[k])));
    y = y < 0x1p-52 ? 0x1p-52 : (y > 1 - 0x1p-52 ? 1 - 0x1p-52 : y);
    ys[k] = y;
    lyy[k * 2 + 0] = log1p(-y);
    lyy[k * 2 + 1] = log(y);
}
__global__ void point_update_kernel(PttView v, const double *__restrict__ ys, const dd *__restrict__ C, float *zs,
                                    float *m_z, float *v_z, AdamConsts adam, int *nonfinite_step, int step)
{
    const int64_t k = (int64_t)blockIdx.x * blockDim.x + threadIdx.x;
    if (k >= v.n - 1) return;
    const int lo = v.lo[k], mid = v.mid[k], hi1 = v.hi1[k];
    const double Hr = dd_diff(C[mid], C[lo]), Hl = dd_diff(C[hi1], C[mid]);
    const double y = ys[k];
    const double zg = y * (1 - y) * (Hl / y - Hr / (1.0 - y));
    if (!isfinite(zg)) atomicCAS(nonfinite_step, 0, step);
    float m = m_z[k], vv = v_z[k], p = zs[k];
    if (adam.first) {
        m = (float)zg;
        vv = (float)(zg * zg);
    } else {
        m = (float)(adam.rm * (double)m + (1 - adam.rm) * zg);
        vv = (float)(adam.rv * (double)vv + (1 - adam.rv) * (zg * zg));
    }
    const double pm = (double)m / adam.m_denom, pv = (double)vv / adam.v_denom;
    double delta = adam.lr * pm / (sqrt(pv) + adam.eps);
    delta = delta < -adam.max_mu ? -adam.max_mu : (delta > adam.max_mu ? adam.max_mu : delta);
    zs[k] = (float)((double)p + delta);
    m_z[k] = m;
    v_z[k] = vv;
}

template <int K>
__global__ void vi_values_finish_kernel(const double *part_ladj, int nchunks, const double *csum, double *row_sums)
{
    __shared__ double smd[4 * K];
    double s[K];
#pragma unroll
    for (int d = 0; d < K; ++d) s[d] = 0.0;
    for (int ch = threadIdx.x; ch < nchunks; ch += blockDim.x)
#pragma unroll
        for (int d = 0; d < K; ++d) s[d] += part_ladj[(size_t)ch * K + d];
    block_sum_vec<K>(s, smd);
#pragma unroll
    for (int d = 0; d < K; ++d)
        if (threadIdx.x == d) {
            row_sums[d * 2 + 1] = s[d];
            row_sums[d * 2 + 0] = csum ? csum[d] : 0.0;
        }
}

}
```

Baseline: 2764.

## Split Monte Carlo draws across workgroups in VI forward-apply and backward-local kernels

Templates the forward apply and backward local kernels on a draws-per-workgroup parameter, so each chunk is processed by several workgroups that each handle a subset of the K draws. Sibling workgroups are laid out chunk-major with a padded stride. The default splits the backward kernel into two-draw groups when K is 6 and leaves the forward kernel unsplit. The aim is smaller per-block shared memory and registers and more blocks in flight, which should raise occupancy and parallelism. The cost is redundant per-chunk work such as topology loads and node index reads, plus extra launched blocks.

```diff
diff --git a/include/polee_hip_debug.h b/include/polee_hip_debug.h
--- a/include/polee_hip_debug.h
+++ b/include/polee_hip_debug.h
@@ -64,6 +64,8 @@
 polee_status polee_debug_fast_log(polee_ctx *ctx, const double *x, int64_t count, double *out);
 polee_status polee_debug_fast_exp(polee_ctx *ctx, const double *x, int64_t count, double *out);
 
+polee_status polee_vi_debug_set_draw_split(polee_vi *vi, int32_t dpw_fwd, int32_t dpw_bwd, int32_t dpw_update);
+
 polee_status polee_debug_gibbs_assignments(polee_gibbs *g, int32_t chain, int32_t *z);
 
 polee_status polee_debug_binomial(polee_ctx *ctx, const int64_t *N, const double *p, int64_t count, uint64_t seed, int64_t *out);
diff --git a/polee_amd/csrc/vi.hip b/polee_amd/csrc/vi.hip
--- a/polee_amd/csrc/vi.hip
+++ b/polee_amd/csrc/vi.hip
@@ -6,6 +6,7 @@
 #include "sampler_internal.hpp"
 
 #include <cmath>
+#include <type_traits>
 
 namespace polee {
 
@@ -174,9 +175,29 @@
     DevBuf<double> d_ygrad, d_xgrad_rows;
     DevBuf<float> d_mug, d_omg, d_alg, d_x_rows;
 
+    int32_t dpw_fwd = 0, dpw_bwd = 0;
+
     NoiseSrc noise() const { return NoiseSrc{d_z0.p, o.seed, K, (int64_t)n - 1}; }
     polee_status one_step(bool apply, bool want_values, bool hook_outputs);
 };
+
+static inline int draw_split_default(int K, int kernel)
+{
+    return kernel == 1 && K == 6 ? 2 : K;
+}
+static inline bool draw_split_offered(int K, int dpw) { return dpw == K || (dpw >= 1 && dpw <= 3 && dpw < K); }
+template <int K, typename F>
+static inline void with_draw_split(int dpw, F &&f)
+{
+    if (dpw == 3 && K > 3)
+        f(std::integral_constant<int, (K > 3 ? 3 : K)>{});
+    else if (dpw == 2 && K > 2)
+        f(std::integral_constant<int, (K > 2 ? 2 : K)>{});
+    else if (dpw == 1 && K > 1)
+        f(std::integral_constant<int, 1>{});
+    else
+        f(std::integral_constant<int, K>{});
+}
 
 template <int K>
 static polee_status vi_step_k(polee_vi *vi, bool apply, bool want_values, bool hook_outputs)
@@ -217,23 +238,27 @@
     } else {
         POLEE_HIP_TRY(ctx, hipMemsetAsync(chunk_f, 0, sizeof(VK<K>), st));
     }
-    if (want_values) {
-        hipLaunchKernelGGL((vi_fwd_apply_kernel<K, YRows, float, true>), dim3(nch_f), dim3(SCAN_THREADS), 0, st, lview, ysrc, chunk_f,
+    const int dpw_f = vi->dpw_fwd ? vi->dpw_fwd : draw_split_default(K, 0);
+    const int dpw_b = vi->dpw_bwd ? vi->dpw_bwd : draw_split_default(K, 1);
+    static const bool sib_far = getenv("POLEE_VI_SPLIT_CONSECUTIVE") != nullptr;
+    const bool sib_near = !sib_far;
+    auto fwd_apply = [&](auto ladj, auto dpw) {
+        constexpr bool LADJ = decltype(ladj)::value;
+        constexpr int DPW = decltype(dpw)::value;
+        const int sib = sib_near ? draw_split_sib(nch_f) : 0;
+        hipLaunchKernelGGL((vi_fwd_apply_kernel<K, YRows, float, LADJ, DPW>), dim3(DrawSplit<K, DPW>::grid(nch_f, sib)), dim3(SCAN_THREADS), 0, st,
+                           lview, ysrc, chunk_f,
                            vi->d_u32.p, vi->d_x.p, vi->d_g.p, eff, (float)o.y_eps, (float)(1.0 - o.y_eps),
                            eff ? vi->d_part_c.p : nullptr, want_values ? vi->d_part_ladj.p : nullptr, nch_f > 1 ? own_f : 0,
                            (const uint32_t *)vi->d_open_ptr.p, (const uint32_t *)vi->d_open_code.p,
                            xwin_here ? (const uint32_t *)vi->ll->d_tslot_ptr.p : nullptr, xwin_here ? (const uint32_t *)vi->ll->d_tslot.p : nullptr,
                            xwin_here ? vi->ll->d_xwin.p : nullptr,
-                           remap && remap->singles_in_g ? (const float *)vi->d_single_leaf.p : nullptr);
-    } else {
-        hipLaunchKernelGGL((vi_fwd_apply_kernel<K, YRows, float, false>), dim3(nch_f), dim3(SCAN_THREADS), 0, st, lview, ysrc, chunk_f,
-                           vi->d_u32.p, vi->d_x.p, vi->d_g.p, eff, (float)o.y_eps, (float)(1.0 - o.y_eps),
-                           eff ? vi->d_part_c.p : nullptr, want_values ? vi->d_part_ladj.p : nullptr, nch_f > 1 ? own_f : 0,
-                           (const uint32_t *)vi->d_open_ptr.p, (const uint32_t *)vi->d_open_code.p,
-                           xwin_here ? (const uint32_t *)vi->ll->d_tslot_ptr.p : nullptr, xwin_here ? (const uint32_t *)vi->ll->d_tslot.p : nullptr,
-                           xwin_here ? vi->ll->d_xwin.p : nullptr,
-                           remap && remap->singles_in_g ? (const float *)vi->d_single_leaf.p : nullptr);
-    }
+                           remap && remap->singles_in_g ? (const float *)vi->d_single_leaf.p : nullptr, nch_f, sib);
+    };
+    if (want_values)
+        with_draw_split<K>(dpw_f, [&](auto dpw) { fwd_apply(std::true_type{}, dpw); });
+    else
+        with_draw_split<K>(dpw_f, [&](auto dpw) { fwd_apply(std::false_type{}, dpw); });
     POLEE_KERNEL_CHECK(ctx);
     if (want_values) POLEE_HIP_TRY(ctx, hipMemsetAsync(vi->d_lp.p, 0, sizeof(double) * PSELL_MAX_K, st));
     {
@@ -286,7 +311,11 @@
         VD<K> *chunk_bu = reinterpret_cast<VD<K> *>(vi->d_chunk_bu.p);
         const BwdArgs<K> ba{lview, vi->d_u32.p, vi->d_g.p, eff, vi->d_csum.p, gp, chunk_bu, vi->d_C.p, (const uint32_t *)vi->d_need.p,
                             (const int32_t *)vi->d_node_start.p, vi->d_H.p};
-        hipLaunchKernelGGL((vi_bwd_local_kernel<K>), dim3(nch_bu), dim3(256), 0, st, ba);
+        with_draw_split<K>(dpw_b, [&](auto dpw) {
+            constexpr int DPW = decltype(dpw)::value;
+            const int sib = sib_near ? draw_split_sib(nch_bu) : 0;
+            hipLaunchKernelGGL((vi_bwd_local_kernel<K, DPW>), dim3(DrawSplit<K, DPW>::grid(nch_bu, sib)), dim3(256), 0, st, ba, nch_bu, sib);
+        });
         if (nm1 > 0) {
             hipLaunchKernelGGL((vi_bwd_spine_kernel<K>), dim3(1), dim3(64 * K), 0, st, chunk_bu, nch_bu);
             hipLaunchKernelGGL((vi_update_k_kernel<K, NoiseSrc>), dim3((unsigned)ceil_div(nm1, 256)), dim3(256), 0, st, view,
@@ -520,6 +549,13 @@
     vi->o = o;
     vi->n = t->n;
     vi->K = o.num_mc_samples;
+    if (const char *e = getenv("POLEE_VI_DRAW_SPLIT")) {
+        int f = 0, b = 0;
+        if (sscanf(e, "%d,%d", &f, &b) == 2) {
+            vi->dpw_fwd = draw_split_offered(vi->K, f) ? f : 0;
+            vi->dpw_bwd = draw_split_offered(vi->K, b) ? b : 0;
+        }
+    }
     ll->profile = o.profile != 0;
     ll->prof_every = o.profile > 1 ? o.profile : 1;
     const size_t n = vi->n, nm1 = std::max<size_t>(n - 1, 1), K = vi->K;
@@ -794,6 +830,19 @@
     return hipMemcpyFromSymbol(out, HIP_SYMBOL(polee::g_vi_stamps), sizeof(unsigned long long) * 4 * 2048 * 8) == hipSuccess ? POLEE_OK : POLEE_ERR_HIP;
 }
 #endif
+
+polee_status polee_vi_debug_set_draw_split(polee_vi *vi, int32_t dpw_fwd, int32_t dpw_bwd, int32_t dpw_update)
+{
+    if (!vi) return fail(nullptr, POLEE_ERR_BAD_ARG, "null handle");
+    for (int32_t dpw : {dpw_fwd, dpw_bwd})
+        if (dpw != 0 && !draw_split_offered(vi->K, dpw))
+            return fail(vi->ctx, POLEE_ERR_BAD_ARG, "draw split %d of %d draws is not instantiated (0, %d, or 3, 2, 1 below it)", dpw, vi->K, vi->K);
+    if (dpw_update != 0 && dpw_update != vi->K)
+        return fail(vi->ctx, POLEE_ERR_BAD_ARG, "the update kernel runs all %d draws of a node on one lane: dpw_update must be 0 or %d", vi->K, vi->K);
+    vi->dpw_fwd = dpw_fwd;
+    vi->dpw_bwd = dpw_bwd;
+    return POLEE_OK;
+}
 
 polee_status polee_vi_export_noise(polee_vi *vi, int32_t step, float *z0)
 {
@@ -887,7 +936,7 @@
         hipLaunchKernelGGL((vi_fwd_apply_kernel<1, LogRows, double, false>), dim3(nch_f), dim3(SCAN_THREADS), 0, st, view, LogRows{vi->d_lyy.p}, chunk_f,
                            vi->d_uleaf.p, vi->d_x.p, vi->d_g.p, vi->d_efflens.p, (float)o.y_eps, (float)(1.0 - o.y_eps),
                            vi->d_part_c.p, (double *)nullptr, 0, (const uint32_t *)nullptr, (const uint32_t *)nullptr,
-                           (const uint32_t *)nullptr, (const uint32_t *)nullptr, (float *)nullptr, (const float *)nullptr);
+                           (const uint32_t *)nullptr, (const uint32_t *)nullptr, (float *)nullptr, (const float *)nullptr, nch_f, 0);
         POLEE_KERNEL_CHECK(ctx);
         return POLEE_OK;
     };
diff --git a/polee_amd/csrc/vi_fused.hpp b/polee_amd/csrc/vi_fused.hpp
--- a/polee_amd/csrc/vi_fused.hpp
+++ b/polee_amd/csrc/vi_fused.hpp
@@ -87,6 +87,36 @@
     }
 };
 
+template <int K, int DPW>
+struct DrawSplit {
+    static_assert(DPW >= 1 && DPW <= K, "draws per workgroup");
+    static constexpr int NG = (K + DPW - 1) / DPW;
+    static constexpr bool REM = K % DPW != 0;
+    __device__ static inline int ld(int d0, int dl) { return REM ? min(d0 + dl, K - 1) : d0 + dl; }
+    __device__ static inline bool on(int d0, int dl) { return !REM || d0 + dl < K; }
+    __device__ static inline bool block(int nch, int sib, int &chunk, int &d0)
+    {
+        if constexpr (NG == 1) {
+            chunk = blockIdx.x;
+            d0 = 0;
+            return true;
+        } else {
+            int grp;
+            if (sib) {
+                grp = blockIdx.x / sib;
+                chunk = blockIdx.x - grp * sib;
+            } else {
+                chunk = blockIdx.x / NG;
+                grp = blockIdx.x - chunk * NG;
+            }
+            d0 = grp * DPW;
+            return chunk < nch;
+        }
+    }
+    static inline unsigned grid(int nch, int sib) { return (unsigned)(NG == 1 ? nch : (sib ? sib : nch) * NG); }
+};
+inline int draw_split_sib(int nch) { return (nch + 7) / 8 * 8; }
+
 template <int K>
 __device__ inline void block_sum_vec(double (&v)[K], double *smem)
 {
@@ -175,12 +205,12 @@
     const double *lyy;
     template <int K>
     __device__ inline double edge_one(uint32_t k, uint32_t left, int d) const { return lyy[((size_t)k * 2 + left) * K + d]; }
-    template <int K>
-    __device__ inline void edge(uint32_t k, uint32_t left, double (&e)[K]) const
+    template <int K, int DPW>
+    __device__ inline void edge(uint32_t k, uint32_t left, int d0, double (&e)[DPW]) const
     {
         const double *p = lyy + ((size_t)k * 2 + left) * K;
 #pragma unroll
-        for (int d = 0; d < K; ++d) e[d] = p[d];
+        for (int d = 0; d < DPW; ++d) e[d] = p[DrawSplit<K, DPW>::ld(d0, d)];
     }
 };
 struct YRows {
@@ -192,14 +222,14 @@
         const double y = clamped_y_pos(y32[(size_t)k * K + d], y_eps, 1.0 - y_eps);
         return fast_log_pos(left ? y : 1.0 - y);
     }
-    template <int K>
-    __device__ inline void edge(uint32_t k, uint32_t left, double (&e)[K]) const
+    template <int K, int DPW>
+    __device__ inline void edge(uint32_t k, uint32_t left, int d0, double (&e)[DPW]) const
     {
         const float *p = y32 + (size_t)k * K;
         const double hi = 1.0 - y_eps;
 #pragma unroll
-        for (int d = 0; d < K; ++d) {
-            const double y = clamped_y_pos(p[d], y_eps, hi);
+        for (int d = 0; d < DPW; ++d) {
+            const double y = clamped_y_pos(p[DrawSplit<K, DPW>::ld(d0, d)], y_eps, hi);
             e[d] = fast_log_pos(left ? y : 1.0 - y);
         }
     }
@@ -209,19 +239,19 @@
 constexpr int FWD_CHUNK = SCAN_THREADS * FWD_ITEMS;
 inline int fwd_num_chunks(int64_t len) { return (int)((len + FWD_CHUNK - 1) / FWD_CHUNK); }
 
-template <int K, typename Src>
-__device__ inline VK<K> tour_value(uint32_t code, const Src &src, VK<K> &edge)
-{
-    VK<K> val;
+template <int K, int DPW, typename Src>
+__device__ inline VK<DPW> tour_value(uint32_t code, const Src &src, int d0, VK<DPW> &edge)
+{
+    VK<DPW> val;
     const uint32_t type = code & 3u;
     if (code & 4u) {
 #pragma unroll
-        for (int d = 0; d < K; ++d) edge.v[d] = 0.0;
+        for (int d = 0; d < DPW; ++d) edge.v[d] = 0.0;
     } else {
-        src.template edge<K>(code >> 4, (code >> 3) & 1u, edge.v);
-    }
-#pragma unroll
-    for (int d = 0; d < K; ++d) val.v[d] = type == TOUR_ENTER ? edge.v[d] : (type == TOUR_EXIT ? -edge.v[d] : 0.0);
+        src.template edge<K, DPW>(code >> 4, (code >> 3) & 1u, d0, edge.v);
+    }
+#pragma unroll
+    for (int d = 0; d < DPW; ++d) val.v[d] = type == TOUR_ENTER ? edge.v[d] : (type == TOUR_EXIT ? -edge.v[d] : 0.0);
     return val;
 }
 
@@ -244,13 +274,25 @@
     VK<K> acc = ScanOps<VK<K>>::zero(), edge;
 #pragma unroll
     for (int j = 0; j < FWD_ITEMS; ++j)
-        if (base + j < v.TL) acc = ScanOps<VK<K>>::add(acc, tour_value<K, Src>(v.tour_code[base + j], lyy, edge));
+        if (base + j < v.TL) acc = ScanOps<VK<K>>::add(acc, tour_value<K, K, Src>(v.tour_code[base + j], lyy, 0, edge));
     VK<K> tot;
     (void)block_exclusive_scan<VK<K>>(acc, smem, &tot);
     if (threadIdx.x == 0) chunk_sums[blockIdx.x] = tot;
 }
 
-template <int K, typename Src, typename UT, bool LADJ>
+template <int K, int DPW>
+__device__ inline VK<DPW> chunk_prefix_draws(const VK<K> *__restrict__ chunk_sums, int chunk, int d0, VK<DPW> *smem)
+{
+    VK<DPW> acc = ScanOps<VK<DPW>>::zero();
+    for (int i = threadIdx.x; i < chunk; i += SCAN_THREADS)
+#pragma unroll
+        for (int d = 0; d < DPW; ++d) acc.v[d] = acc.v[d] + chunk_sums[i].v[DrawSplit<K, DPW>::ld(d0, d)];
+    VK<DPW> tot;
+    (void)block_exclusive_scan<VK<DPW>>(acc, smem, &tot);
+    return tot;
+}
+
+template <int K, typename Src, typename UT, bool LADJ, int DPW = K>
 __global__ __launch_bounds__(SCAN_THREADS) void vi_fwd_apply_kernel(PttView v, Src lyy,
                                                                    const VK<K> *__restrict__ chunk_offsets,
                                                                    UT *__restrict__ uleaf, float *__restrict__ xs,
@@ -263,20 +305,23 @@
                                                                    const uint32_t *__restrict__ tslot_ptr,
                                                                    const uint32_t *__restrict__ tslot,
                                                                    float *__restrict__ xwin,
-                                                                   const float *__restrict__ single_cnt)
-{
-    __shared__ VK<K> smem[SCAN_THREADS / 64];
-    __shared__ double smd[4 * K];
-    __shared__ double spre[K];
-    __shared__ double smd2[LADJ ? 4 * K : 1];
+                                                                   const float *__restrict__ single_cnt, int nch, int sib)
+{
+    using DS = DrawSplit<K, DPW>;
+    __shared__ VK<DPW> smem[SCAN_THREADS / 64];
+    __shared__ double smd[4 * DPW];
+    __shared__ double spre[DPW];
+    __shared__ double smd2[LADJ ? 4 * DPW : 1];
     constexpr int XW_INLINE = 12, XW_DEFER = 48;
     __shared__ uint32_t xw_tid[XW_DEFER];
-    __shared__ float xw_val[XW_DEFER][K];
+    __shared__ float xw_val[XW_DEFER][DPW];
     __shared__ int xw_count;
+    int chunk, d0;
+    if (!DS::block(nch, sib, chunk, d0)) return;
     if (xwin && threadIdx.x == 0) xw_count = 0;
     if (xwin) __syncthreads();
-    const int64_t base = (int64_t)blockIdx.x * FWD_CHUNK + (int64_t)threadIdx.x * FWD_ITEMS;
-    VK<K> w[FWD_ITEMS];
+    const int64_t base = (int64_t)chunk * FWD_CHUNK + (int64_t)threadIdx.x * FWD_ITEMS;
+    VK<DPW> w[FWD_ITEMS];
     uint32_t code[FWD_ITEMS];
     int tgt[FWD_ITEMS];
 #pragma unroll
@@ -288,17 +333,17 @@
     const int lane = threadIdx.x & 63;
     uint32_t ob = 0, oe = 0;
     if (open_ptr) {
-        ob = open_ptr[blockIdx.x];
-        oe = open_ptr[blockIdx.x + 1];
+        ob = open_ptr[chunk];
+        oe = open_ptr[chunk + 1];
     }
     const int wave = threadIdx.x >> 6;
     const uint32_t ocode0 = ob + lane < oe ? open_code[ob + lane] : (4u | TOUR_LEAF);
-    VK<K> acc = ScanOps<VK<K>>::zero();
+    VK<DPW> acc = ScanOps<VK<DPW>>::zero();
     float inv_l_[FWD_ITEMS], sc_[FWD_ITEMS];
     int ltid[FWD_ITEMS];
 #pragma unroll
     for (int j = 0; j < FWD_ITEMS; ++j) {
-        acc = ScanOps<VK<K>>::add(acc, tour_value<K, Src>(code[j], lyy, w[j]));
+        acc = ScanOps<VK<DPW>>::add(acc, tour_value<K, DPW, Src>(code[j], lyy, d0, w[j]));
         const bool leaf = (code[j] & 3u) == TOUR_LEAF && base + j < v.TL;
         ltid[j] = leaf ? (v.leaf_tid ? v.leaf_tid[tgt[j]] : tgt[j]) : 0;
         inv_l_[j] = leaf && efflens ? 1.0f / efflens[ltid[j]] : 0.0f;
@@ -307,38 +352,46 @@
     VI_STAMP(0, 1);
     if (open_ptr) {
 #pragma unroll
-        for (int dd_ = 0; dd_ < (K + 3) / 4; ++dd_) {
-            const int d = wave + 4 * dd_;
-            if (d < K) {
+        for (int dd_ = 0; dd_ < (DPW + 3) / 4; ++dd_) {
+            const int dl = wave + 4 * dd_;
+            if (dl < DPW) {
+                const int d = DS::ld(d0, dl);
                 double pre = (ocode0 & 4u) ? 0.0 : lyy.template edge_one<K>(ocode0 >> 4, (ocode0 >> 3) & 1u, d);
                 for (uint32_t e = ob + 64 + lane; e < oe; e += 64) {
                     const uint32_t oc = open_code[e];
                     pre += lyy.template edge_one<K>(oc >> 4, (oc >> 3) & 1u, d);
                 }
                 pre = wave_inclusive_scan<double>(pre);
-                if (lane == 63) spre[d] = pre;
+                if (lane == 63) spre[dl] = pre;
             }
         }
     }
     VI_STAMP(0, 2);
-    VK<K> tot;
-    VK<K> off = block_exclusive_scan<VK<K>>(acc, smem, &tot);
+    VK<DPW> tot;
+    VK<DPW> off = block_exclusive_scan<VK<DPW>>(acc, smem, &tot);
     VI_STAMP(0, 3);
     if (open_ptr) {
 #pragma unroll
-        for (int d = 0; d < K; ++d) off.v[d] += spre[d];
+        for (int d = 0; d < DPW; ++d) off.v[d] += spre[d];
     } else {
-        off = ScanOps<VK<K>>::add(own_prefix ? chunk_prefix<VK<K>>(chunk_offsets, blockIdx.x, smem) : chunk_offsets[blockIdx.x], off);
-    }
-    double pc[K], pl[K];
-#pragma unroll
-    for (int d = 0; d < K; ++d) pc[d] = pl[d] = 0.0;
+        VK<DPW> co;
+        if (own_prefix) {
+            co = chunk_prefix_draws<K, DPW>(chunk_offsets, chunk, d0, smem);
+        } else {
+#pragma unroll
+            for (int d = 0; d < DPW; ++d) co.v[d] = chunk_offsets[chunk].v[DS::ld(d0, d)];
+        }
+        off = ScanOps<VK<DPW>>::add(co, off);
+    }
+    double pc[DPW], pl[DPW];
+#pragma unroll
+    for (int d = 0; d < DPW; ++d) pc[d] = pl[d] = 0.0;
 #pragma unroll
     for (int j = 0; j < FWD_ITEMS; ++j) {
         const uint32_t tj = code[j] & 3u;
 #pragma unroll
-        for (int d = 0; d < K; ++d) off.v[d] = tj == TOUR_ENTER ? off.v[d] + w[j].v[d] : (tj == TOUR_EXIT ? off.v[d] - w[j].v[d] : off.v[d]);
-        const VK<K> &inc = off;
+        for (int d = 0; d < DPW; ++d) off.v[d] = tj == TOUR_ENTER ? off.v[d] + w[j].v[d] : (tj == TOUR_EXIT ? off.v[d] - w[j].v[d] : off.v[d]);
+        const VK<DPW> &inc = off;
         if (base + j < v.TL) {
             const uint32_t type = code[j] & 3u;
             if (type == TOUR_LEAF) {
@@ -346,15 +399,19 @@
                 const int tid = ltid[j];
                 const float inv_l = inv_l_[j];
                 const float sc = sc_[j];
-#pragma unroll
-                for (int d = 0; d < K; ++d) {
+                float xv[DPW];
+#pragma unroll
+                for (int d = 0; d < DPW; ++d) {
                     const double u = fast_exp(inc.v[d] + w[j].v[d]);
-                    uleaf[(size_t)pos * K + d] = (UT)u;
                     float x = (float)u;
                     x = (float)fmax((double)x, 1e-16);
                     x = fminf(fmaxf(x, clamp_lo), clamp_hi);
-                    xs[(size_t)tid * K + d] = x;
-                    g[(size_t)tid * K + d] = sc != 0.0f ? sc / x : 0.0f;
+                    xv[d] = x;
+                    if (DS::on(d0, d)) {
+                        uleaf[(size_t)pos * K + d0 + d] = (UT)u;
+                        xs[(size_t)tid * K + d0 + d] = x;
+                        g[(size_t)tid * K + d0 + d] = sc != 0.0f ? sc / x : 0.0f;
+                    }
                     pc[d] += (double)(x * inv_l);
                 }
                 if (xwin) {
@@ -364,18 +421,19 @@
                     if (q >= 0 && q < XW_DEFER) {
                         xw_tid[q] = (uint32_t)tid;
 #pragma unroll
-                        for (int d = 0; d < K; ++d) xw_val[q][d] = xs[(size_t)tid * K + d];
+                        for (int d = 0; d < DPW; ++d) xw_val[q][d] = xv[d];
                     } else {
                         for (uint32_t e = sb; e < se; ++e) {
-                            float *w = xwin + (size_t)tslot[e] * K;
-#pragma unroll
-                            for (int d = 0; d < K; ++d) w[d] = xs[(size_t)tid * K + d];
+                            float *w = xwin + (size_t)tslot[e] * K + d0;
+#pragma unroll
+                            for (int d = 0; d < DPW; ++d)
+                                if (DS::on(d0, d)) w[d] = xv[d];
                         }
                     }
                 }
             } else if (LADJ && type == TOUR_ENTER) {
 #pragma unroll
-                for (int d = 0; d < K; ++d) pl[d] += inc.v[d];
+                for (int d = 0; d < DPW; ++d) pl[d] += inc.v[d];
             }
         }
     }
@@ -384,28 +442,28 @@
         const int cnt = min(xw_count, XW_DEFER);
         for (int q = 0; q < cnt; ++q) {
             const uint32_t tid = xw_tid[q], sb = tslot_ptr[tid], se = tslot_ptr[tid + 1];
-            for (uint32_t e = sb * K + threadIdx.x; e < se * K; e += SCAN_THREADS) {
-                const uint32_t slot = e / K, d = e - slot * K;
-                xwin[(size_t)tslot[slot] * K + d] = xw_val[q][d];
+            for (uint32_t e = sb * DPW + threadIdx.x; e < se * DPW; e += SCAN_THREADS) {
+                const uint32_t slot = e / DPW, d = e - slot * DPW;
+                if (DS::on(d0, (int)d)) xwin[(size_t)tslot[slot] * K + d0 + d] = xw_val[q][d];
             }
         }
     }
     VI_STAMP(0, 4);
     if (part_c || LADJ) {
 #pragma unroll
-        for (int d = 0; d < K; ++d) {
+        for (int d = 0; d < DPW; ++d) {
             const double a = wave_inclusive_scan<double>(pc[d]);
             const double b = LADJ ? wave_inclusive_scan<double>(pl[d]) : 0.0;
             if (lane == 63) {
-                smd[wave * K + d] = a;
-                if (LADJ) smd2[wave * K + d] = b;
+                smd[wave * DPW + d] = a;
+                if (LADJ) smd2[wave * DPW + d] = b;
             }
         }
         __syncthreads();
-        if ((int)threadIdx.x < K) {
+        if ((int)threadIdx.x < DPW && DS::on(d0, (int)threadIdx.x)) {
             const int d = threadIdx.x;
-            if (part_c) part_c[(size_t)blockIdx.x * K + d] = ((smd[d] + smd[K + d]) + smd[2 * K + d]) + smd[3 * K + d];
-            if (LADJ) part_ladj[(size_t)blockIdx.x * K + d] = ((smd2[d] + smd2[K + d]) + smd2[2 * K + d]) + smd2[3 * K + d];
+            if (part_c) part_c[(size_t)chunk * K + d0 + d] = ((smd[d] + smd[DPW + d]) + smd[2 * DPW + d]) + smd[3 * DPW + d];
+            if (LADJ) part_ladj[(size_t)chunk * K + d0 + d] = ((smd2[d] + smd2[DPW + d]) + smd2[2 * DPW + d]) + smd2[3 * DPW + d];
         }
     }
     VI_STAMP(0, 5);
@@ -685,10 +743,10 @@
     csum_finish_block<K>(part_c, nparts, out, smd);
 }
 
-template <int K>
+template <int K, int DPW>
 __device__ inline void bwd_leaf(const PttView &v, int64_t pos, const float *__restrict__ uleaf, const float *__restrict__ g,
                                 const float *__restrict__ efflens, const double *c, const double *inv_c, const GenePrior &gp,
-                                double (&a)[K])
+                                int d0, double (&a)[DPW])
 {
     const int tid = v.leaf_tid ? v.leaf_tid[pos] : (int)pos;
     const float inv_lf = efflens ? 1.0f / efflens[tid] : 0.0f;
@@ -699,15 +757,16 @@
         kg = gene >= 0 ? gp.gene_k[gene] : 0;
     }
 #pragma unroll
-    for (int d = 0; d < K; ++d) {
+    for (int dl = 0; dl < DPW; ++dl) {
+        const int d = DrawSplit<K, DPW>::ld(d0, dl);
         double xg = (double)g[(size_t)tid * K + d];
-        if (efflens) xg -= (double)nl * inv_c[d];
+        if (efflens) xg -= (double)nl * inv_c[dl];
         if (gp.gene_of) {
-            const double cc = c[d], inv_l = (double)inv_lf;
+            const double cc = c[dl], inv_l = (double)inv_lf;
             const double xlg = kg > 1 ? -(double)(kg - 1) / gp.gene_c[(size_t)gene * K + d] : 0.0;
             xg += xlg * (inv_l / cc) + inv_l * (gp.M / (cc * cc));
         }
-        a[d] = (double)uleaf[(size_t)pos * K + d] * xg;
+        a[dl] = (double)uleaf[(size_t)pos * K + d] * xg;
     }
 }
 
@@ -717,37 +776,40 @@
     return dd{s, (a - (s - bb)) + (b - bb)};
 }
 
-template <int K>
-__global__ __launch_bounds__(256) void vi_bwd_local_kernel(BwdArgs<K> B)
-{
+template <int K, int DPW = K>
+__global__ __launch_bounds__(256) void vi_bwd_local_kernel(BwdArgs<K> B, int nch, int sib)
+{
+    using DS = DrawSplit<K, DPW>;
     constexpr int CH = bu_ch<K>(), LPT = CH / 256;
-    __shared__ dd P[(CH + 1) * K];
-    __shared__ VD<K> wtot[4];
+    __shared__ dd P[(CH + 1) * DPW];
+    __shared__ VD<DPW> wtot[4];
     const PttView &v = B.v;
+    int chunk, d0;
+    if (!DS::block(nch, sib, chunk, d0)) return;
     const int lane = threadIdx.x & 63, wave = threadIdx.x >> 6;
-    double c[K], inv_c[K];
-#pragma unroll
-    for (int d = 0; d < K; ++d) {
-        c[d] = B.efflens ? B.csum[d] : 1.0;
-        inv_c[d] = B.efflens ? B.csum[K + d] : 1.0;
+    double c[DPW], inv_c[DPW];
+#pragma unroll
+    for (int d = 0; d < DPW; ++d) {
+        c[d] = B.efflens ? B.csum[DS::ld(d0, d)] : 1.0;
+        inv_c[d] = B.efflens ? B.csum[K + DS::ld(d0, d)] : 1.0;
     }
     VI_STAMP(1, 0);
-    const int64_t base = (int64_t)blockIdx.x * CH, p0 = base + (int64_t)threadIdx.x * LPT;
+    const int64_t base = (int64_t)chunk * CH, p0 = base + (int64_t)threadIdx.x * LPT;
     const int64_t end = min(base + CH, (int64_t)v.n), nm1 = (int64_t)v.n - 1;
     const bool exp0 = p0 <= v.n && ((B.need[p0 >> 5] >> (p0 & 31)) & 1u);
     const bool exp1 = LPT == 2 && p0 + 1 <= v.n && ((B.need[(p0 + 1) >> 5] >> ((p0 + 1) & 31)) & 1u);
-    double a[LPT][K];
+    double a[LPT][DPW];
 #pragma unroll
     for (int j = 0; j < LPT; ++j) {
         if (p0 + j < v.n)
-            bwd_leaf<K>(v, p0 + j, B.uleaf, B.g, B.efflens, c, inv_c, B.gp, a[j]);
+            bwd_leaf<K, DPW>(v, p0 + j, B.uleaf, B.g, B.efflens, c, inv_c, B.gp, d0, a[j]);
         else
 #pragma unroll
-            for (int d = 0; d < K; ++d) a[j][d] = 0.0;
+            for (int d = 0; d < DPW; ++d) a[j][d] = 0.0;
     }
     constexpr int PRE = LPT;
     const uint32_t vz = threadIdx.x >> 12;
-    const int32_t k0 = B.node_start[blockIdx.x + vz] + (int32_t)threadIdx.x, k1 = B.node_start[blockIdx.x + 1 + vz];
+    const int32_t k0 = B.node_start[chunk + vz] + (int32_t)threadIdx.x, k1 = B.node_start[chunk + 1 + vz];
     int32_t kp[PRE];
     int plo[PRE], pmid[PRE], phi[PRE];
 #pragma unroll
@@ -758,53 +820,55 @@
         pmid[i] = in ? v.mid[kp[i]] : 0;
         phi[i] = in ? v.hi1[kp[i]] : 0;
     }
-    VD<K> s;
-#pragma unroll
-    for (int d = 0; d < K; ++d) {
+    VD<DPW> s;
+#pragma unroll
+    for (int d = 0; d < DPW; ++d) {
         s.v[d] = dd_make(a[0][d]);
         if constexpr (LPT == 2) s.v[d] = two_sum(a[0][d], a[1][d]);
     }
     VI_STAMP(1, 1);
-    const VD<K> inc = wave_inclusive_scan<VD<K>>(s);
+    const VD<DPW> inc = wave_inclusive_scan<VD<DPW>>(s);
     VI_STAMP(1, 2);
     if (lane == 63) wtot[wave] = inc;
     __syncthreads();
-    VD<K> off = wave_shift_up_one<VD<K>>(inc);
-    for (int w = 0; w < wave; ++w) off = ScanOps<VD<K>>::add(wtot[w], off);
-#pragma unroll
-    for (int d = 0; d < K; ++d) P[(size_t)(threadIdx.x * LPT) * K + d] = off.v[d];
+    VD<DPW> off = wave_shift_up_one<VD<DPW>>(inc);
+    for (int w = 0; w < wave; ++w) off = ScanOps<VD<DPW>>::add(wtot[w], off);
+#pragma unroll
+    for (int d = 0; d < DPW; ++d) P[(size_t)(threadIdx.x * LPT) * DPW + d] = off.v[d];
     if (exp0)
 #pragma unroll
-        for (int d = 0; d < K; ++d) B.C[(size_t)p0 * K + d] = off.v[d];
+        for (int d = 0; d < DPW; ++d)
+            if (DS::on(d0, d)) B.C[(size_t)p0 * K + d0 + d] = off.v[d];
     if constexpr (LPT == 2) {
         const int64_t p1 = p0 + 1;
 #pragma unroll
-        for (int d = 0; d < K; ++d) {
+        for (int d = 0; d < DPW; ++d) {
             const dd o1 = dd_add(off.v[d], dd_make(a[0][d]));
-            P[(size_t)(threadIdx.x * LPT + 1) * K + d] = o1;
-            if (exp1) B.C[(size_t)p1 * K + d] = o1;
+            P[(size_t)(threadIdx.x * LPT + 1) * DPW + d] = o1;
+            if (exp1 && DS::on(d0, d)) B.C[(size_t)p1 * K + d0 + d] = o1;
         }
     }
     if (threadIdx.x == 255) {
-        VD<K> tot;
-#pragma unroll
-        for (int d = 0; d < K; ++d) {
-            tot.v[d] = dd_add(off.v[d], s.v[d]);
-            P[(size_t)CH * K + d] = tot.v[d];
-        }
-        B.chunk_tot[blockIdx.x] = tot;
+#pragma unroll
+        for (int d = 0; d < DPW; ++d) {
+            const dd tot = dd_add(off.v[d], s.v[d]);
+            P[(size_t)CH * DPW + d] = tot;
+            if (DS::on(d0, d)) B.chunk_tot[chunk].v[d0 + d] = tot;
+        }
     }
     VI_STAMP(1, 3);
     __syncthreads();
     VI_STAMP(1, 4);
     auto node = [&](int32_t k, int lo, int mid, int hi1) {
         if (hi1 > end) return;
-        const dd *Plo = P + (size_t)(lo - base) * K, *Pmid = P + (size_t)(mid - base) * K, *Phi = P + (size_t)(hi1 - base) * K;
-#pragma unroll
-        for (int d = 0; d < K; ++d) {
+        const dd *Plo = P + (size_t)(lo - base) * DPW, *Pmid = P + (size_t)(mid - base) * DPW, *Phi = P + (size_t)(hi1 - base) * DPW;
+#pragma unroll
+        for (int d = 0; d < DPW; ++d) {
             const dd pm = Pmid[d];
-            B.H[(size_t)d * nm1 + k] = (float)dd_diff(pm, Plo[d]);
-            B.H[(size_t)(K + d) * nm1 + k] = (float)dd_diff(Phi[d], pm);
+            if (DS::on(d0, d)) {
+                B.H[(size_t)(d0 + d) * nm1 + k] = (float)dd_diff(pm, Plo[d]);
+                B.H[(size_t)(K + d0 + d) * nm1 + k] = (float)dd_diff(Phi[d], pm);
+            }
         }
     };
 #pragma unroll
```

Measured after the change: 2795, median of 6. 1.01x the previous value.
